# google-research/snap

Measured on AMD Instinct MI355X. Metric: localization_scenes_per_sec, higher is better.
Workload: dtype f32 (tensors, accumulation, every non-GEMM op); conv / dense products on the bf16 matrix cores: operands split into 2 bf16 parts, 3 part products per MAC, ~2^-17 per product; 1 GPU; C2: 8 scenes/GPU, 4 StreetView views @512px + aerial, 128x128x60 voxel BEV @0.2m, ResNet-50 encoders, 10001 pose hypotheses; scenes_per_gpu=8, batches_in_flight=2, global_batch=8, parallelism=scene-sharded x1, no data-path collective, mode=inference forward (BEVLocalizer.apply, train=False)

## Files before the change

### include/snap_hip.h

```cpp
#ifndef SNAP_HIP_H_
#define SNAP_HIP_H_

#include <stddef.h>
#include <stdint.h>

#ifdef __cplusplus
extern "C" {
#endif

typedef enum SnapStatus {
  SNAP_OK = 0,
  SNAP_ERR_BAD_SHAPE = -1,
  SNAP_ERR_UNSUPPORTED = -2,
  SNAP_ERR_NULL = -3,
  SNAP_ERR_LAUNCH = -4,
  SNAP_ERR_WORKSPACE = -5
} SnapStatus;

int snap_abi_version(void);
const char* snap_status_string(int status);
const char* snap_build_arch(void);

enum { SNAP_PRO_NONE = 0, SNAP_PRO_AFFINE = 1, SNAP_PRO_GN_RELU = 2,
       SNAP_PRO_RELU_GN = 3, SNAP_PRO_RELU = 4 };
enum { SNAP_EPI_BIAS = 1, SNAP_EPI_RELU = 2, SNAP_EPI_RESIDUAL = 4,
       SNAP_EPI_UPSAMPLE2X_ADD = 8, SNAP_EPI_ROWMASK = 16,
       SNAP_EPI_GELU = 32  };

typedef struct SnapConvDesc {
  int32_t N, H, W, Cin, Cin_stride;
  int32_t KH, KW, stride, pad_t, pad_l;
  int32_t Ho, Wo, Cout, Cout_stride;
  int32_t prologue;
  int32_t epilogue;
  float in_scale, in_shift;
  int32_t tile_hint;
} SnapConvDesc;

int snap_conv2d_nhwc_f32(const SnapConvDesc* desc, const float* x, const float* w,
                         float* y, const float* gn_mu, const float* gn_sc,
                         const float* gn_beta, const float* bias,
                         const float* residual, const float* up_prev,
                         const uint8_t* row_mask, void* stream);

typedef struct SnapConvExtras {
  const int32_t* rows_in;
  const int32_t* rows_out;
  const int32_t* row_count;
  float* gn_partial;
  size_t gn_partial_bytes;
  int32_t gn_partial_relu;
  void* workspace;
  size_t workspace_bytes;
  const void* w_bf16;
  size_t w_bf16_bytes;
  int32_t w_split_parts;
  int32_t w_split_root;
  float* gn_partial2;
  size_t gn_partial2_bytes;
  int32_t gn_partial2_done;
  int32_t x_presplit;
  int32_t ps_tile;
  int32_t ps_res_init;
  int32_t bk_hint;
  int32_t tune_flags;
  int32_t gn_partial_rows;
  int32_t w_half;
  int32_t x_half;
  void* y_half;
  const float* gnb_x;
  const float* gnb_mu;
  const float* gnb_rstd;
  const float* gnb_gamma;
  const float* gnb_beta;
  int32_t gnb_mode;
} SnapConvExtras;
#define SNAP_TUNE_NO_HALO 1
#define SNAP_TUNE_NO_PLAIN 8
#define SNAP_TUNE_RS_NSPLIT_SHIFT 4
int32_t snap_conv2d_presplit_tile_rows(const SnapConvDesc* desc, int32_t ps_tile);
size_t snap_conv2d_presplit_gn_partial_bytes(const SnapConvDesc* desc, int32_t ps_tile);
size_t snap_conv2d_presplit_workspace_bytes(const SnapConvDesc* desc, int32_t ps_tile);
int32_t snap_conv2d_presplit_supported(const SnapConvDesc* desc);
int snap_gn_norm_split_f32(const float* y, const float* partial, int32_t N, int32_t HW, int32_t C,
                           int32_t groups, float eps, int32_t tile_rows, const float* gamma,
                           const float* beta, void* out, float* mu, float* sc, void* stream);
int snap_presplit_f32(const float* x, int64_t rows, int32_t C, void* out, void* stream);

int snap_conv2d_nhwc_ex_f32(const SnapConvDesc* desc, const float* x, const float* w,
                            float* y, const float* gn_mu, const float* gn_sc,
                            const float* gn_beta, const float* bias,
                            const float* residual, const float* up_prev,
                            const uint8_t* row_mask, const SnapConvExtras* extras,
                            void* stream);
size_t snap_conv2d_packed_weights_split_root_bytes(int32_t Cout, int32_t parts);
int snap_conv2d_pack_weights_split_root_bf16(const float* w , int32_t Cout,
                                             int32_t parts, void* out, size_t out_bytes,
                                             void* stream);
size_t snap_conv2d_packed_weights_bytes(int32_t taps, int32_t Cin, int32_t Cout);
int snap_conv2d_pack_weights_bf16(const float* w, int32_t taps, int32_t Cin, int32_t Cout,
                                  void* out, size_t out_bytes, void* stream);
int snap_conv2d_pack_weights_f16(const float* w, int32_t taps, int32_t Cin, int32_t Cout,
                                 void* out, size_t out_bytes, void* stream);
size_t snap_conv2d_packed_weights_split_bytes(int32_t taps, int32_t Cin, int32_t Cout,
                                              int32_t parts);
int snap_conv2d_pack_weights_split_bf16(const float* w, int32_t taps, int32_t Cin, int32_t Cout,
                                        int32_t parts, void* out, size_t out_bytes, void* stream);
typedef struct SnapPackItem {
  const float* w;
  void* out;
  int32_t taps, Cin, Cout, block_begin;
} SnapPackItem;
int32_t snap_conv2d_pack_weights_split_blocks(int32_t taps, int32_t Cin, int32_t Cout);
int32_t snap_conv2d_pack_weights_blocks(int32_t taps, int32_t Cin, int32_t Cout);
int snap_conv2d_pack_weights_multi_bf16(const SnapPackItem* items, int32_t n_items,
                                        int32_t total_blocks, void* stream);
int snap_conv2d_pack_weights_multi_f16(const SnapPackItem* items, int32_t n_items,
                                       int32_t total_blocks, void* stream);
int snap_conv2d_pack_weights_split_multi_bf16(const SnapPackItem* items, int32_t n_items,
                                              int32_t total_blocks, int32_t parts, void* stream);

int snap_interpolate_nd_f32(const float* array, const int32_t* size, int32_t n, int32_t D,
                            const uint8_t* valid_array, const float* points, int64_t K,
                            float* values, uint8_t* valid, void* stream);
int snap_expectation_nd_f32(const float* pdf, int64_t rows, const int32_t* size, int32_t n,
                            float* out, void* stream);
int snap_occupancy_ray_features_f32(const float* hits, const float* origins, const uint8_t* ray_mask,
                                    int64_t num_rays, int32_t num_samples, float margin, const float* points,
                                    int64_t num_points, int32_t B, const float* volume,
                                    const uint8_t* volume_valid, int32_t X, int32_t Y, int32_t Z, int32_t D,
                                    float cell_size, float* out_points, uint8_t* out_labels,
                                    uint8_t* out_ray_valid, float* features, uint8_t* valid, void* stream);
int32_t snap_occupancy_head_supported(int32_t D, int32_t h1, int32_t h2);
int snap_occupancy_head_f32(const float* hits, const float* origins, const uint8_t* ray_mask, int64_t num_rays,
                            int32_t num_samples, float margin, const float* points, int64_t num_points, int32_t B,
                            const float* volume, const uint8_t* volume_valid, int32_t X, int32_t Y, int32_t Z,
                            int32_t D, float cell_size, const float* w0, const float* b0, int32_t h1,
                            const float* w1, const float* b1, int32_t h2, const float* w_out,
                            const float* b_out, float* out_points, uint8_t* out_labels, uint8_t* out_ray_valid,
                            float* logits, uint8_t* valid, void* stream);
int32_t snap_occupancy_features_vjp_chunk(void);
size_t snap_occupancy_features_vjp_workspace_bytes(int64_t num_points, int32_t B, int32_t X, int32_t Y, int32_t Z,
                                                   int32_t D);
int snap_occupancy_ray_features_vjp_f32(const float* hits, const float* origins, const uint8_t* ray_mask,
                                        int64_t num_rays, int32_t num_samples, float margin, const float* points,
                                        int64_t num_points, int32_t B, int32_t X, int32_t Y, int32_t Z, int32_t D,
                                        float cell_size, const float* d_features, float* d_volume, void* workspace,
                                        size_t workspace_bytes, void* stream);

int snap_semantic_embed_f32(const uint8_t* rasters, int64_t M, int32_t N, const int32_t* idx_road,
                            int32_t nr, const int32_t* idx_other, int32_t no,
                            const float* table_road, const float* table_other, int32_t E,
                            float* out, void* stream);
int snap_semantic_onehot_f32(const uint8_t* rasters, int64_t M, int32_t N, const int32_t* idx_road,
                             int32_t nr, const int32_t* idx_other, int32_t no, float* onehot,
                             int32_t KP, void* stream);

int snap_layer_norm_f32(const float* x, const float* gamma, const float* beta, float* y,
// ... 433 lines not shown
```

### snap_amd/_lib.py

```python
import ctypes
import os

_HERE = os.path.dirname(os.path.abspath(__file__))
LIB_PATH = os.environ.get('SNAP_HIP_LIB') or os.path.join(_HERE, 'lib', 'libsnap_hip.so')

c_int = ctypes.c_int32
c_i64 = ctypes.c_int64
c_u64 = ctypes.c_uint64
c_float = ctypes.c_float
c_size = ctypes.c_size_t
ptr = ctypes.c_void_p


class SnapConvDesc(ctypes.Structure):
  _fields_ = [
      ('N', c_int), ('H', c_int), ('W', c_int), ('Cin', c_int),
      ('Cin_stride', c_int),
      ('KH', c_int), ('KW', c_int), ('stride', c_int), ('pad_t', c_int),
      ('pad_l', c_int),
      ('Ho', c_int), ('Wo', c_int), ('Cout', c_int), ('Cout_stride', c_int),
      ('prologue', c_int), ('epilogue', c_int),
      ('in_scale', c_float), ('in_shift', c_float), ('tile_hint', c_int),
  ]


class SnapConvExtras(ctypes.Structure):
  _fields_ = [
      ('rows_in', ptr), ('rows_out', ptr), ('row_count', ptr), ('gn_partial', ptr),
      ('gn_partial_bytes', c_size), ('gn_partial_relu', c_int),
      ('workspace', ptr), ('workspace_bytes', c_size),
      ('w_bf16', ptr), ('w_bf16_bytes', c_size), ('w_split_parts', c_int), ('w_split_root', c_int),
      ('gn_partial2', ptr), ('gn_partial2_bytes', c_size), ('gn_partial2_done', c_int),
      ('x_presplit', c_int), ('ps_tile', c_int), ('ps_res_init', c_int),
      ('bk_hint', c_int), ('tune_flags', c_int), ('gn_partial_rows', c_int), ('w_half', c_int), ('x_half', c_int), ('y_half', ptr),
      ('gnb_x', ptr), ('gnb_mu', ptr), ('gnb_rstd', ptr), ('gnb_gamma', ptr), ('gnb_beta', ptr), ('gnb_mode', c_int),
  ]


class SnapLiftDesc(ctypes.Structure):
  _fields_ = [
      ('B', c_int), ('V', c_int), ('h', c_int), ('w', c_int), ('C', c_int),
      ('feature_dim', c_int), ('num_bins', c_int), ('N', c_int), ('K', c_int),
      ('fisheye', c_int), ('out_stride', c_int),
      ('depth_min', c_float), ('depth_max', c_float),
      ('max_view_distance', c_float),
      ('weighted', c_int), ('use_variance', c_int), ('add_minmax', c_int),
      ('grid_y', c_int), ('grid_z', c_int), ('valid_rows_only', c_int), ('out_split', c_int),
      ('class_rows', c_int), ('tune_flags', c_int),
  ]


SIGNATURES = {
    'snap_abi_version': (c_int, []),
    'snap_status_string': (ctypes.c_char_p, [c_int]),
    'snap_build_arch': (ctypes.c_char_p, []),
    'snap_conv2d_nhwc_f32': (
        c_int,
        [ctypes.POINTER(SnapConvDesc), ptr, ptr, ptr, ptr, ptr, ptr, ptr, ptr,
         ptr, ptr, ptr],
    ),
    'snap_conv2d_nhwc_ex_f32': (
        c_int,
        [ctypes.POINTER(SnapConvDesc), ptr, ptr, ptr, ptr, ptr, ptr, ptr, ptr,
         ptr, ptr, ctypes.POINTER(SnapConvExtras), ptr],
    ),
    'snap_conv2d_gn_partial_bytes': (c_size, [ctypes.POINTER(SnapConvDesc)]),
    'snap_conv2d_workspace_bytes': (c_size, [ctypes.POINTER(SnapConvDesc)]),
    'snap_conv2d_tile_rows': (c_int, [ctypes.POINTER(SnapConvDesc)]),
    'snap_conv2d_pack_weights_blocks': (c_int, [c_int, c_int, c_int]),
    'snap_conv2d_pack_weights_multi_bf16': (c_int, [ptr, c_int, c_int, ptr]),
    'snap_conv2d_pack_weights_multi_f16': (c_int, [ptr, c_int, c_int, ptr]),
    'snap_conv2d_stationary_kind': (c_int, [ctypes.POINTER(SnapConvDesc), c_int]),
    'snap_conv2d_tile_rows_ex': (c_int, [ctypes.POINTER(SnapConvDesc), c_int]),
    'snap_conv2d_gn_partial_bytes_ex': (c_size, [ctypes.POINTER(SnapConvDesc), c_int]),
    'snap_conv2d_splitk_gn_partial_bytes': (c_size, [ctypes.POINTER(SnapConvDesc)]),
    'snap_conv2d_presplit_tile_rows': (c_int, [ctypes.POINTER(SnapConvDesc), c_int]),
    'snap_conv2d_presplit_gn_partial_bytes': (c_size, [ctypes.POINTER(SnapConvDesc), c_int]),
    'snap_conv2d_presplit_workspace_bytes': (c_size, [ctypes.POINTER(SnapConvDesc), c_int]),
    'snap_conv2d_presplit_supported': (c_int, [ctypes.POINTER(SnapConvDesc)]),
    'snap_gn_norm_split_f32': (
        c_int, [ptr, ptr, c_int, c_int, c_int, c_int, c_float, c_int, ptr, ptr, ptr, ptr, ptr, ptr]),
    'snap_presplit_f32': (c_int, [ptr, c_i64, c_int, ptr, ptr]),
    'snap_interpolate_nd_f32': (c_int, [ptr, ptr, c_int, c_int, ptr, ptr, c_i64, ptr, ptr, ptr]),
    'snap_expectation_nd_f32': (c_int, [ptr, c_i64, ptr, c_int, ptr, ptr]),
    'snap_occupancy_ray_features_f32': (
        c_int, [ptr, ptr, ptr, c_i64, c_int, c_float, ptr, c_i64, c_int, ptr, ptr, c_int, c_int, c_int, c_int,
                c_float, ptr, ptr, ptr, ptr, ptr, ptr]),
    'snap_occupancy_head_supported': (c_int, [c_int, c_int, c_int]),
    'snap_occupancy_head_f32': (
        c_int, [ptr, ptr, ptr, c_i64, c_int, c_float, ptr, c_i64, c_int, ptr, ptr, c_int, c_int, c_int, c_int,
                c_float, ptr, ptr, c_int, ptr, ptr, c_int, ptr, ptr, ptr, ptr, ptr, ptr, ptr, ptr]),
    'snap_occupancy_features_vjp_chunk': (c_int, []),
    'snap_occupancy_features_vjp_workspace_bytes': (c_size, [c_i64, c_int, c_int, c_int, c_int, c_int]),
    'snap_occupancy_ray_features_vjp_f32': (
        c_int, [ptr, ptr, ptr, c_i64, c_int, c_float, ptr, c_i64, c_int, c_int, c_int, c_int, c_int, c_float,
                ptr, ptr, ptr, c_size, ptr]),
    'snap_semantic_embed_f32': (
        c_int, [ptr, c_i64, c_int, ptr, c_int, ptr, c_int, ptr, ptr, c_int, ptr, ptr]),
    'snap_semantic_onehot_f32': (c_int, [ptr, c_i64, c_int, ptr, c_int, ptr, c_int, ptr, c_int, ptr]),
    'snap_voting_fft_workspace_bytes': (c_size, [c_int] * 6),
    'snap_voting_fft_f32': (
        c_int, [ptr, ptr, ptr, ptr, ptr, c_int, c_int, c_int, c_int, c_int, c_int, c_float, c_int, ptr, c_size,
                ptr, ptr]),
    'snap_voting_fft_rotated_f32': (
        c_int, [ptr, ptr, ptr, c_float, ptr, ptr, c_int, c_int, c_int, c_int, c_int, c_float, ptr, c_size, ptr, ptr]),
    'snap_stack_templates_f32': (c_int, [ptr, ptr, c_int, c_int, c_int, c_int, c_int, ptr]),
    'snap_stack_templates_rhwd_f32': (c_int, [ptr, ptr, c_int, c_int, c_int, c_int, c_int, ptr]),
    'snap_pack_stacked_templates_split_bf16': (c_int, [ptr, c_int, c_int, c_int, c_int, c_int, ptr, c_size, ptr]),
    'snap_layer_norm_f32': (c_int, [ptr, ptr, ptr, ptr, c_i64, c_int, c_float, ptr]),
    'snap_attention_bf16_f32': (c_int, [ptr, ptr, c_int, c_int, c_int, c_int, c_float, ptr]),
    'snap_layer_norm_bf16out_f32': (c_int, [ptr, ptr, ptr, ptr, c_i64, c_int, c_float, ptr]),
    'snap_attention_bf16out_f32': (c_int, [ptr, ptr, c_int, c_int, c_int, c_int, c_float, ptr]),
    'snap_attention_bf16io': (c_int, [ptr, ptr, c_int, c_int, c_int, c_int, c_float, ptr]),
    'snap_attention_lse_bf16_f32': (c_int, [ptr, ptr, ptr, c_int, c_int, c_int, c_int, c_float, ptr]),
    'snap_attention_bwd_bf16_f32': (
        c_int, [ptr, ptr, ptr, ptr, ptr, ptr, c_int, c_int, c_int, c_int, c_float, ptr]),
    'snap_layer_norm_bwd_workspace_bytes': (c_size, [c_i64, c_int]),
    'snap_layer_norm_bwd_f32': (
# ... 258 lines not shown
```

### snap_amd/csrc/conv_common.h

```cpp
#ifndef SNAP_CSRC_CONV_COMMON_H_
#define SNAP_CSRC_CONV_COMMON_H_

#include <stdio.h>
#include <stdlib.h>

#include "common.h"

namespace snapconv {
struct ConvArgs {
  SnapConvDesc d;
  const float* x;
  const float* w;
  float* y;
  const float* gn_mu;
  const float* gn_sc;
  const float* gn_beta;
  const float* bias;
  const float* residual;
  const float* up_prev;
  const uint8_t* row_mask;
  const int32_t* rows_in;
  const int32_t* rows_out;
  const int32_t* row_count;
  float* kpartial;
  size_t kpartial_bytes;
  int ksplit;
  int slabs_per_split;
  int tiles_per_split;
  float* gn_partial;
  float* gn_partial2;
  int32_t* gn_partial2_done;
  int gn_relu;
  int gn_rows32;
  int gn_slabs;
  int M;
  int K;
  int ctiles;
  int nk;
  int ncol;
  int bk;
  int no_halo;
  int no_plain;
  int rs_nsplit;
  const void* w_bf16;
  int cin8;
  int half;
  const void* x_half;
  void* y_half;
  const void* x_ps;
  int ps_tile;
  int ps_res_init;
  int ps_parts;
  const float* gnb_x;
  const float* gnb_mu;
  const float* gnb_rstd;
  const float* gnb_gamma;
  const float* gnb_beta;
  int gnb_mode;
};

int launch_bf16(ConvArgs a, hipStream_t s);
int launch_split(ConvArgs a, int parts, hipStream_t s);
int launch_split_root(ConvArgs a, int parts, hipStream_t s);
int launch_ps(ConvArgs a, hipStream_t s);
int stationary_kind(const SnapConvDesc& d, int parts, bool row_lists);
int launch_rs(ConvArgs a, hipStream_t s);
int launch_bs(ConvArgs a, hipStream_t s);
int launch_root_ws(const ConvArgs& a, hipStream_t s);
struct PsTile { int bm, bn, nt; };
PsTile ps_choose_tile(int64_t M, int64_t N, int force);
int ps_ksplit(int64_t M, int Cout, int64_t nk, int bm, int bn, size_t kpartial_bytes);

}

namespace {
using snapconv::ConvArgs;

template <int PRO>
__device__ __forceinline__ float apply_pro(float v, float mu, float sc, float beta, float s,
                                           float t) {
  if constexpr (PRO == SNAP_PRO_AFFINE) return v * s + t;
  if constexpr (PRO == SNAP_PRO_GN_RELU) return snap_relu((v - mu) * sc + beta);
  if constexpr (PRO == SNAP_PRO_RELU_GN) return (snap_relu(v) - mu) * sc + beta;
  if constexpr (PRO == SNAP_PRO_RELU) return snap_relu(v);
  return v;
}

typedef __attribute__((address_space(3))) void lds_void_t;
typedef const __attribute__((address_space(1))) void cglobal_void_t;

__device__ __attribute__((aligned(64))) const float kZeroChunk[16] = {0.f};

__device__ __forceinline__ float snap_gelu_tanh(float x) {
  const float u = 0.7978845608028654f * (x + 0.044715f * x * x * x);
  return x / (1.0f + __expf(-2.0f * u));
}

template <int BM, int BN, bool DUAL = false, int NT = 256, bool SKIP_RES = false, int OUTH = 0, bool GNB = false>
__device__ __forceinline__ void conv_epilogue(const ConvArgs& a,
                                              f32x16 (&acc)[BM / (NT / 4)][BN / 64],
                                              float* smem, int m0, int n0, int Meff, int row_t,
                                              int split) {
  constexpr int WR = NT / 128;
  constexpr int TM = BM / (32 * WR), TN = BN / 64;
  const SnapConvDesc& d = a.d;
  const int tid = threadIdx.x;
  const int lane = tid & 63;
  const int wid = tid >> 6;
  const int wr = wid >> 1, wc = wid & 1;
  const int l31 = lane & 31, lhi = lane >> 5;
  const int HoWo = d.Ho * d.Wo;
  const int epi = d.epilogue;
  const int Hp = d.Ho >> 1, Wp = d.Wo >> 1;
  constexpr int Q = BN / 4;
  constexpr int PER_THREAD = (32 * WR * Q) / NT;
  const bool want_stats = a.gn_partial != nullptr && a.ksplit == 1;
  const int n_first = m0 / HoWo;
  const int m_split = (n_first + 1) * HoWo;
  float gs1[2][4] = {{0.f, 0.f, 0.f, 0.f}, {0.f, 0.f, 0.f, 0.f}};
  float gs2[2][4] = {{0.f, 0.f, 0.f, 0.f}, {0.f, 0.f, 0.f, 0.f}};
  const bool want_relu_too = DUAL && want_stats;
  float hs1[2][4] = {{0.f, 0.f, 0.f, 0.f}, {0.f, 0.f, 0.f, 0.f}};
  float hs2[2][4] = {{0.f, 0.f, 0.f, 0.f}, {0.f, 0.f, 0.f, 0.f}};
  f32x4 vb_mu[2], vb_rs[2], vb_g = {0.f, 0.f, 0.f, 0.f}, vb_b = {0.f, 0.f, 0.f, 0.f};
  const bool gnb = GNB && want_stats && a.gnb_mode != 0;
  if constexpr (GNB) {
    vb_mu[0] = vb_mu[1] = vb_rs[0] = vb_rs[1] = vb_g;
    const int colq = n0 + 4 * (tid % Q);
    if (gnb && colq < d.Cout) {
      vb_g = *reinterpret_cast<const f32x4*>(a.gnb_gamma + colq);
      vb_b = *reinterpret_cast<const f32x4*>(a.gnb_beta + colq);
#pragma unroll
      for (int sl = 0; sl < 2; ++sl) {
        const int64_t so = (int64_t)min(n_first + sl, d.N - 1) * d.Cout + colq;
        vb_mu[sl] = *reinterpret_cast<const f32x4*>(a.gnb_mu + so);
        vb_rs[sl] = *reinterpret_cast<const f32x4*>(a.gnb_rstd + so);
      }
    }
  }
#pragma unroll
  for (int h = 0; h < TM; ++h) {
    if (h > 0) __syncthreads();
#pragma unroll
    for (int j = 0; j < TN; ++j)
#pragma unroll
      for (int r = 0; r < 16; ++r) {
        const int ri = (r & 3) + 8 * (r >> 2) + 4 * lhi;
        smem[(wr * 32 + ri) * BN + wc * (BN / 2) + j * 32 + l31] = acc[h][j][r];
      }
    __syncthreads();
#pragma unroll
    for (int it = 0; it < PER_THREAD; ++it) {
      const int idx = tid + NT * it;
      const int row = idx / Q, q = idx - row * Q;
      const int m = m0 + (row >> 5) * (BM / WR) + h * 32 + (row & 31);
      const int col = n0 + 4 * q;
      if (m >= Meff || col >= d.Cout) continue;
      f32x4 v = *reinterpret_cast<const f32x4*>(smem + row * BN + 4 * q);
      if (a.ksplit > 1) {
        *reinterpret_cast<f32x4*>(a.kpartial + ((int64_t)split * a.M + m) * d.Cout + col) = v;
        continue;
      }
      const int64_t o = (int64_t)(a.rows_out ? a.rows_out[m] : m) * d.Cout_stride + col;
      if (epi & SNAP_EPI_BIAS) {
        const f32x4 bb = *reinterpret_cast<const f32x4*>(a.bias + col);
#pragma unroll
        for (int e = 0; e < 4; ++e) v[e] += bb[e];
      }
      if (!SKIP_RES && (epi & SNAP_EPI_RESIDUAL)) {
        const f32x4 rr = *reinterpret_cast<const f32x4*>(a.residual + o);
#pragma unroll
        for (int e = 0; e < 4; ++e) v[e] += rr[e];
      }
      if (epi & SNAP_EPI_UPSAMPLE2X_ADD) {
        const int n = m / HoWo;
        const int rr = m - n * HoWo;
        const int ho = rr / d.Wo;
        const int wo = rr - ho * d.Wo;
        const float sh = (ho + 0.5f) * 0.5f - 0.5f;
        const float sw = (wo + 0.5f) * 0.5f - 0.5f;
        const float fh = floorf(sh), fw = floorf(sw);
        const float wh_hi = sh - fh, wh_lo = 1.f - wh_hi;
        const float ww_hi = sw - fw, ww_lo = 1.f - ww_hi;
        const int h0 = min(max((int)fh, 0), Hp - 1), h1 = min(max((int)fh + 1, 0), Hp - 1);
        const int w0 = min(max((int)fw, 0), Wp - 1), w1 = min(max((int)fw + 1, 0), Wp - 1);
        const int64_t base = (int64_t)n * Hp * Wp;
        const f32x4 p00 = *reinterpret_cast<const f32x4*>(
            a.up_prev + (base + (int64_t)h0 * Wp + w0) * d.Cout_stride + col);
        const f32x4 p01 = *reinterpret_cast<const f32x4*>(
            a.up_prev + (base + (int64_t)h0 * Wp + w1) * d.Cout_stride + col);
        const f32x4 p10 = *reinterpret_cast<const f32x4*>(
            a.up_prev + (base + (int64_t)h1 * Wp + w0) * d.Cout_stride + col);
        const f32x4 p11 = *reinterpret_cast<const f32x4*>(
            a.up_prev + (base + (int64_t)h1 * Wp + w1) * d.Cout_stride + col);
#pragma unroll
        for (int e = 0; e < 4; ++e) {
          const float c0 = p00[e] * wh_lo + p10[e] * wh_hi;
          const float c1 = p01[e] * wh_lo + p11[e] * wh_hi;
          v[e] += c0 * ww_lo + c1 * ww_hi;
        }
      }
      if (epi & SNAP_EPI_RELU) {
#pragma unroll
        for (int e = 0; e < 4; ++e) v[e] = snap_relu(v[e]);
      }
      if (epi & SNAP_EPI_GELU) {
#pragma unroll
        for (int e = 0; e < 4; ++e) v[e] = snap_gelu_tanh(v[e]);
      }
      if ((epi & SNAP_EPI_ROWMASK) && a.row_mask[m] == 0) v = f32x4{0.f, 0.f, 0.f, 0.f};
      if constexpr (OUTH == 0) {
        *reinterpret_cast<f32x4*>(a.y + o) = v;
      } else {
        if (a.y) *reinterpret_cast<f32x4*>(a.y + o) = v;
        if constexpr (OUTH == 1) {
          typedef __bf16 bf16x4_t __attribute__((ext_vector_type(4)));
          *reinterpret_cast<bf16x4_t*>(static_cast<__bf16*>(a.y_half) + o) = __builtin_convertvector(v, bf16x4_t);
        } else {
          typedef _Float16 f16x4_t __attribute__((ext_vector_type(4)));
          *reinterpret_cast<f16x4_t*>(static_cast<_Float16*>(a.y_half) + o) = __builtin_convertvector(v, f16x4_t);
        }
      }
      if (GNB && gnb) {
        const int sl = m >= m_split ? 1 : 0;
        const f32x4 xv = *reinterpret_cast<const f32x4*>(a.gnb_x + (int64_t)m * d.Cout + col);
#pragma unroll
        for (int e = 0; e < 4; ++e) {
          float xh, dyp;
          if (a.gnb_mode == SNAP_PRO_GN_RELU) {
            xh = (xv[e] - vb_mu[sl][e]) * vb_rs[sl][e];
            dyp = (xh * vb_g[e] + vb_b[e] > 0.f) ? v[e] : 0.f;
          } else {
            xh = (fmaxf(xv[e], 0.f) - vb_mu[sl][e]) * vb_rs[sl][e];
            dyp = v[e];
          }
          gs1[sl][e] += dyp;
          gs2[sl][e] += dyp * xh;
        }
      } else if (want_stats) {
        const int sl = m >= m_split ? 1 : 0;
#pragma unroll
        for (int e = 0; e < 4; ++e) {
          const float t = a.gn_relu ? snap_relu(v[e]) : v[e];
          gs1[sl][e] += t;
          gs2[sl][e] += t * t;
          if constexpr (DUAL) {
            const float r = snap_relu(v[e]);
            hs1[sl][e] += r;
            hs2[sl][e] += r * r;
          }
        }
      }
    }
  }
  if (want_stats) {
    constexpr int RG = NT / Q;
    const int q = tid % Q, rg = tid / Q;
    for (int pass = 0; pass < (want_relu_too ? 2 : 1); ++pass) {
    float* const dst_partial = pass ? a.gn_partial2 : a.gn_partial;
    __syncthreads();
#pragma unroll
    for (int sl = 0; sl < 2; ++sl)
#pragma unroll
      for (int e = 0; e < 4; ++e) {
        smem[((rg * 2 + sl) * BN + 4 * q + e) * 2 + 0] = pass ? hs1[sl][e] : gs1[sl][e];
        smem[((rg * 2 + sl) * BN + 4 * q + e) * 2 + 1] = pass ? hs2[sl][e] : gs2[sl][e];
      }
    __syncthreads();
    for (int i = tid; i < 2 * BN; i += NT) {
      const int sl = i / BN, c = i - sl * BN;
      const int col = n0 + c;
      const int n = n_first + sl;
      const bool live = col < d.Cout && n < d.N && (sl == 0 || (m0 + BM > m_split && m_split < Meff));
      if (!live) continue;
      float t1 = 0.f, t2 = 0.f;
#pragma unroll
      for (int r = 0; r < RG; ++r) {
        t1 += smem[((r * 2 + sl) * BN + c) * 2 + 0];
        t2 += smem[((r * 2 + sl) * BN + c) * 2 + 1];
      }
      const int slab = row_t - (int)(((int64_t)n * HoWo) / BM);
      float* o = dst_partial + (((int64_t)n * a.gn_slabs + slab) * d.Cout + col) * 2;
      o[0] = t1;
      o[1] = t2;
    }
    }
  }
}

__global__ __launch_bounds__(256) void splitk_reduce_kernel(
    const float* __restrict__ partial, int S, int64_t M, int Cout, int Cout_stride, int epi,
    const float* __restrict__ bias, const float* __restrict__ residual,
    const uint8_t* __restrict__ row_mask, float* __restrict__ y) {
  const int Q = Cout >> 2;
  const int64_t i = (int64_t)blockIdx.x * blockDim.x + threadIdx.x;
  if (i >= M * Q) return;
  const int64_t m = i / Q;
  const int col = 4 * (int)(i - m * Q);
  f32x4 v = *reinterpret_cast<const f32x4*>(partial + m * Cout + col);
  int s = 1;
  for (; s + 3 < S; s += 4) {
    f32x4 t[4];
#pragma unroll
    for (int u = 0; u < 4; ++u)
      t[u] = *reinterpret_cast<const f32x4*>(partial + ((int64_t)(s + u) * M + m) * Cout + col);
#pragma unroll
    for (int u = 0; u < 4; ++u)
#pragma unroll
      for (int e = 0; e < 4; ++e) v[e] += t[u][e];
  }
  for (; s < S; ++s) {
    const f32x4 t = *reinterpret_cast<const f32x4*>(partial + ((int64_t)s * M + m) * Cout + col);
#pragma unroll
    for (int e = 0; e < 4; ++e) v[e] += t[e];
  }
  const int64_t o = m * Cout_stride + col;
  if (epi & SNAP_EPI_BIAS) {
    const f32x4 bb = *reinterpret_cast<const f32x4*>(bias + col);
#pragma unroll
    for (int e = 0; e < 4; ++e) v[e] += bb[e];
  }
  if (epi & SNAP_EPI_RESIDUAL) {
    const f32x4 rr = *reinterpret_cast<const f32x4*>(residual + o);
#pragma unroll
    for (int e = 0; e < 4; ++e) v[e] += rr[e];
  }
  if (epi & SNAP_EPI_RELU) {
#pragma unroll
    for (int e = 0; e < 4; ++e) v[e] = snap_relu(v[e]);
  }
  if (epi & SNAP_EPI_GELU) {
#pragma unroll
    for (int e = 0; e < 4; ++e) v[e] = snap_gelu_tanh(v[e]);
  }
  if ((epi & SNAP_EPI_ROWMASK) && row_mask[m] == 0) v = f32x4{0.f, 0.f, 0.f, 0.f};
  *reinterpret_cast<f32x4*>(y + o) = v;
}

__global__ __launch_bounds__(256) void splitk_reduce_stats_kernel(
    const float* __restrict__ partial, int S, int64_t M, int Cout, int epi,
    const float* __restrict__ bias, const float* __restrict__ residual,
    const uint8_t* __restrict__ row_mask, float* __restrict__ y, int HoWo, int N, int gn_slabs,
    int gn_relu, float* __restrict__ gn_partial) {
  __shared__ float red[256 * 16];
  const int Q = Cout >> 2;
  const int QW = Q < 256 ? Q : 256;
  const int PW = 256 / QW;
  const int tq = threadIdx.x % QW, tp = threadIdx.x / QW;
  const int64_t m0 = (int64_t)blockIdx.x * 32;
  const int n_first = (int)(m0 / HoWo);
  const int64_t m_split = (int64_t)(n_first + 1) * HoWo;
  for (int q0 = 0; q0 < Q; q0 += QW) {
    const int q = q0 + tq;
    const int col = 4 * q;
    float s1[2][4] = {{0.f, 0.f, 0.f, 0.f}, {0.f, 0.f, 0.f, 0.f}};
    float s2[2][4] = {{0.f, 0.f, 0.f, 0.f}, {0.f, 0.f, 0.f, 0.f}};
    if (q < Q && tp < PW) {
      constexpr int RB = 8;
      for (int r0 = tp; r0 < 32; r0 += RB * PW) {
        f32x4 v[RB];
        bool ok[RB];
#pragma unroll
        for (int k = 0; k < RB; ++k) {
          const int64_t m = m0 + r0 + k * PW;
          ok[k] = r0 + k * PW < 32 && m < M;
          v[k] = *reinterpret_cast<const f32x4*>(partial + (ok[k] ? m : m0) * Cout + col);
        }
        for (int sp = 1; sp < S; ++sp) {
          f32x4 t[RB];
#pragma unroll
          for (int k = 0; k < RB; ++k)
            t[k] = *reinterpret_cast<const f32x4*>(partial + ((int64_t)sp * M + (ok[k] ? m0 + r0 + k * PW : m0)) * Cout + col);
#pragma unroll
          for (int k = 0; k < RB; ++k)
#pragma unroll
            for (int e = 0; e < 4; ++e) v[k][e] += t[k][e];
        }
        f32x4 bb = {0.f, 0.f, 0.f, 0.f};
        if (epi & SNAP_EPI_BIAS) bb = *reinterpret_cast<const f32x4*>(bias + col);
        f32x4 rr[RB];
        if (epi & SNAP_EPI_RESIDUAL) {
#pragma unroll
          for (int k = 0; k < RB; ++k)
            rr[k] = *reinterpret_cast<const f32x4*>(residual + (ok[k] ? m0 + r0 + k * PW : m0) * Cout + col);
        }
#pragma unroll
        for (int k = 0; k < RB; ++k) {
          if (!ok[k]) continue;
          const int64_t m = m0 + r0 + k * PW;
          const int64_t o = m * Cout + col;
          if (epi & SNAP_EPI_BIAS) {
#pragma unroll
            for (int e = 0; e < 4; ++e) v[k][e] += bb[e];
          }
          if (epi & SNAP_EPI_RESIDUAL) {
#pragma unroll
            for (int e = 0; e < 4; ++e) v[k][e] += rr[k][e];
          }
          if (epi & SNAP_EPI_RELU) {
#pragma unroll
            for (int e = 0; e < 4; ++e) v[k][e] = snap_relu(v[k][e]);
          }
          if (epi & SNAP_EPI_GELU) {
#pragma unroll
            for (int e = 0; e < 4; ++e) v[k][e] = snap_gelu_tanh(v[k][e]);
          }
          if ((epi & SNAP_EPI_ROWMASK) && row_mask[m] == 0) v[k] = f32x4{0.f, 0.f, 0.f, 0.f};
          *reinterpret_cast<f32x4*>(y + o) = v[k];
          const int sl = m >= m_split ? 1 : 0;
#pragma unroll
          for (int e = 0; e < 4; ++e) {
            const float t = gn_relu ? snap_relu(v[k][e]) : v[k][e];
            s1[sl][e] += t;
            s2[sl][e] += t * t;
          }
        }
      }
    }
    __syncthreads();
#pragma unroll
    for (int sl = 0; sl < 2; ++sl)
#pragma unroll
      for (int e = 0; e < 4; ++e) {
        red[threadIdx.x * 16 + sl * 8 + e] = s1[sl][e];
        red[threadIdx.x * 16 + sl * 8 + 4 + e] = s2[sl][e];
      }
    __syncthreads();
    if (tp == 0 && q < Q) {
#pragma unroll
      for (int sl = 0; sl < 2; ++sl) {
        const int n = n_first + sl;
        const bool live = n < N && (sl == 0 || (m0 + 32 > m_split && m_split < M));
        if (!live) continue;
        const int slab = (int)(blockIdx.x - (((int64_t)n * HoWo) >> 5));
        float* o = gn_partial + (((int64_t)n * gn_slabs + slab) * Cout + col) * 2;
#pragma unroll
        for (int e = 0; e < 4; ++e) {
          float t1 = 0.f, t2 = 0.f;
          for (int pp = 0; pp < PW; ++pp) {
            t1 += red[(pp * QW + tq) * 16 + sl * 8 + e];
            t2 += red[(pp * QW + tq) * 16 + sl * 8 + 4 + e];
          }
          o[2 * e] = t1;
          o[2 * e + 1] = t2;
        }
      }
    }
  }
}

inline int launch_splitk_reduce(const ConvArgs& a, hipStream_t s) {
  if (a.gn_partial) {
    if (!a.gn_rows32 || (a.d.Cout & 3) || (256 % ((a.d.Cout >> 2) < 256 ? (a.d.Cout >> 2) : 256)) != 0)
      return SNAP_ERR_UNSUPPORTED;
    hipLaunchKernelGGL(splitk_reduce_stats_kernel, dim3((unsigned)snap_cdiv((int64_t)a.M, 32)), dim3(256), 0, s,
                       (const float*)a.kpartial, a.ksplit, (int64_t)a.M, a.d.Cout, a.d.epilogue, a.bias,
                       a.residual, a.row_mask, a.y, a.d.Ho * a.d.Wo, a.d.N, (a.d.Ho * a.d.Wo) / 32 + 2,
                       a.gn_relu, a.gn_partial);
  } else {
    const int64_t total4 = (int64_t)a.M * (a.d.Cout / 4);
    hipLaunchKernelGGL(splitk_reduce_kernel, dim3((unsigned)snap_cdiv(total4, 256)), dim3(256), 0, s,
                       (const float*)a.kpartial, a.ksplit, (int64_t)a.M, a.d.Cout, a.d.Cout_stride,
                       a.d.epilogue, a.bias, a.residual, a.row_mask, a.y);
  }
  SNAP_CHECK_LAUNCH();
  return SNAP_OK;
}

constexpr int64_t splitk_max_tiles() { return 384; }
constexpr int splitk_target() { return 768; }

struct TileChoice { int bm, bn; };
inline int hint_tile(int h) { return h % 1000000; }
inline int hint_mode(int h) { return h / 1000000; }
inline int64_t desc_k(const SnapConvDesc& d) { return (int64_t)d.KH * d.KW * d.Cin; }
inline TileChoice choose_tile(int64_t M, int64_t N, int forced, int64_t K) {
  forced = hint_tile(forced);
  const int64_t kMin = 512;
  const bool n_wide_ok = N > 64 && !(N % 128 != 0 && N % 128 <= 64);
  if (forced != 128128 && forced != 128064 && forced != 64128 && forced != 64064) forced = 0;
  if (forced == 128128 || (!forced && n_wide_ok && snap_cdiv(M, 128) * snap_cdiv(N, 128) >= kMin))
    return {128, 128};
  if (!forced && n_wide_ok && K >= 2304 && M >= 128) return {128, 128};
  const int64_t t64128 = snap_cdiv(M, 64) * snap_cdiv(N, 128);
  if (!forced && n_wide_ok && N >= 512 && K >= 1024 && t64128 >= kMin) return {64, 128};
  if (forced == 128064 || (!forced && snap_cdiv(M, 128) * snap_cdiv(N, 64) >= kMin)) return {128, 64};
  if (forced == 64128 || (!forced && n_wide_ok && N >= 512 && t64128 >= kMin)) return {64, 128};
  if (!forced && n_wide_ok && K >= 1024 && t64128 >= 256) return {64, 128};
  return {64, 64};
}

}

#endif
```

### snap_amd/csrc/conv_igemm.hip

```cpp
#include "conv_common.h"

namespace {

template <int BM, int BN, bool VEC, int PRO, int BK, bool DMA = false>
__device__ __forceinline__ void conv_igemm_body(const ConvArgs& a) {
  constexpr int AS = BM + 2;
  constexpr int TM = BM / 64;
  constexpr int TN = BN / 64;
  constexpr int QPR = BK / 4;
  constexpr int RPP = 256 / QPR;
  constexpr int AROWS = BM / RPP;
  constexpr int SRPP = 256 / BK;
  constexpr int AELEMS = BM / SRPP;
  constexpr int BQ = BN / 4;
  constexpr int BROWS_PER_PASS = 256 / BQ;
  constexpr int BPASS = BK / BROWS_PER_PASS;

  constexpr int kDmaStages = 3;
  constexpr int kSlabFloats = DMA ? kDmaStages * (BK * BM + BK * BN) : 2 * BK * AS + 2 * BK * BN;
  constexpr int kStageFloats = 64 * BN;
  constexpr int kSmemFloats = kSlabFloats > kStageFloats ? kSlabFloats : kStageFloats;
  __shared__ __attribute__((aligned(16))) float smem[kSmemFloats];
  float* const As0 = smem;
  float* const Bs0 = smem + 2 * BK * AS;
// ... 246 lines not shown
          const int R = wr * (BM / 2) + i * 32 + l31;
          const int pq = (lhi * 2 + h) ^ ((R >> 2) & 3);
          av[i][h] = *reinterpret_cast<const f32x4*>(as + 4 * (R * 4 + pq));
          if constexpr (PRO == SNAP_PRO_RELU) {
#pragma unroll
            for (int e = 0; e < 4; ++e) av[i][h][e] = snap_relu(av[i][h][e]);
          }
        }
      float bv[2][TN];
#pragma unroll
      for (int jn = 0; jn < TN; ++jn) bv[0][jn] = bs[(8 * lhi) * BN + wc * (BN / 2) + jn * 32 + l31];
#pragma unroll
      for (int j = 0; j < BK / 2; ++j) {
        const int cu = j & 1, nx = cu ^ 1;
        if (j + 1 < BK / 2) {
#pragma unroll
          for (int jn = 0; jn < TN; ++jn)
            bv[nx][jn] = bs[(8 * lhi + j + 1) * BN + wc * (BN / 2) + jn * 32 + l31];
        }
#pragma unroll
        for (int i = 0; i < TM; ++i)
#pragma unroll
          for (int jn = 0; jn < TN; ++jn)
            acc[i][jn] = __builtin_amdgcn_mfma_f32_32x32x2f32(av[i][j >> 2][j & 3], bv[cu][jn], acc[i][jn], 0, 0, 0);
      }
      __builtin_amdgcn_sched_group_barrier(0x100, 2 * TM + TN, 0);
#pragma unroll
      for (int j = 0; j < BK / 2; ++j) {
        if (j + 1 < BK / 2) __builtin_amdgcn_sched_group_barrier(0x100, TN, 0);
        __builtin_amdgcn_sched_group_barrier(0x008, TM * TN, 0);
      }
    }
    __syncthreads();
  } else {
  load_slab(kt_begin);
  advance();
  store_slab(0);
  __syncthreads();

  for (int kt = kt_begin; kt < kt_end; ++kt) {
    const int cur = (kt - kt_begin) & 1;
    const bool more = kt + 1 < kt_end;
    if (more) {
      load_slab(kt + 1);
      advance();
    }
    const float* as = As0 + cur * (BK * AS);
    const float* bs = Bs0 + cur * (BK * BN);
    float av[2][TM], bv[2][TN];
#pragma unroll
    for (int i = 0; i < TM; ++i) av[0][i] = as[lhi * AS + wr * (BM / 2) + i * 32 + l31];
#pragma unroll
    for (int j = 0; j < TN; ++j) bv[0][j] = bs[lhi * BN + wc * (BN / 2) + j * 32 + l31];
#pragma unroll
    for (int kk = 0; kk < BK / 2; ++kk) {
      const int cu = kk & 1, nx = cu ^ 1;
      if (kk + 1 < BK / 2) {
#pragma unroll
        for (int i = 0; i < TM; ++i)
          av[nx][i] = as[(2 * (kk + 1) + lhi) * AS + wr * (BM / 2) + i * 32 + l31];
#pragma unroll
        for (int j = 0; j < TN; ++j)
          bv[nx][j] = bs[(2 * (kk + 1) + lhi) * BN + wc * (BN / 2) + j * 32 + l31];
      }
#pragma unroll
      for (int i = 0; i < TM; ++i)
#pragma unroll
        for (int j = 0; j < TN; ++j)
          acc[i][j] =
              __builtin_amdgcn_mfma_f32_32x32x2f32(av[cu][i], bv[cu][j], acc[i][j], 0, 0, 0);
    }
    __builtin_amdgcn_sched_group_barrier(0x100, TM + TN, 0);
#pragma unroll
    for (int kk = 0; kk < BK / 2; ++kk) {
      if (kk + 1 < BK / 2) __builtin_amdgcn_sched_group_barrier(0x100, TM + TN, 0);
      __builtin_amdgcn_sched_group_barrier(0x008, TM * TN, 0);
    }
    if (more) store_slab(cur ^ 1);
    __syncthreads();
  }

  }

  conv_epilogue<BM, BN>(a, acc, smem, m0, n0, Meff, row_t, split);
}


template <int BM, int BN, bool VEC, int PRO, int BK>
__global__ __launch_bounds__(256) void conv_igemm_kernel(const ConvArgs a) {
  conv_igemm_body<BM, BN, VEC, PRO, BK>(a);
}
template <int BM, int BN, bool VEC, int PRO, int BK>
__global__ __launch_bounds__(256) __attribute__((amdgpu_waves_per_eu(4, 4)))
void conv_igemm_kernel_occ4(const ConvArgs a) {
  conv_igemm_body<BM, BN, VEC, PRO, BK>(a);
}
template <int BM, int BN, int PRO>
__global__ __launch_bounds__(256) void conv_igemm_kernel_dma(const ConvArgs a) {
  conv_igemm_body<BM, BN, true, PRO, 16, true>(a);
}

template <int BM, int BN, bool VEC, int PRO, int BK>
int launch(ConvArgs a, hipStream_t s) {
  if (VEC) {
    a.ctiles = (a.d.Cin + BK - 1) / BK;
    a.nk = a.d.KH * a.d.KW * a.ctiles;
  } else {
    a.ctiles = 0;
    a.nk = (a.K + BK - 1) / BK;
  }
  const int64_t nrow = snap_cdiv(a.M, BM);
  a.ncol = (int)snap_cdiv(a.d.Cout, BN);
  a.gn_slabs = (a.d.Ho * a.d.Wo) / BM + 2;
  int64_t nblocks = snap_cdiv(nrow, 8) * 8 * a.ncol;
  if (nblocks > 0x7fffffffLL) return SNAP_ERR_BAD_SHAPE;
  a.ksplit = 1;
  a.tiles_per_split = (int)nblocks;
  a.slabs_per_split = a.nk;
  const int64_t tiles = nrow * a.ncol;
  const int target = splitk_target();
  if (a.kpartial && target > 0 && tiles <= splitk_max_tiles() && a.nk >= 16 && !a.rows_in &&
      !a.rows_out && !a.row_count && !a.gn_partial &&
      !(a.d.epilogue & SNAP_EPI_UPSAMPLE2X_ADD)) {
    int64_t S = (target + tiles - 1) / tiles;
    S = S < a.nk / 8 ? S : a.nk / 8;
    const int64_t fit = (int64_t)(a.kpartial_bytes / ((size_t)a.M * a.d.Cout * sizeof(float)));
    S = S < fit ? S : fit;
    if (S >= 2) {
      a.slabs_per_split = (int)((a.nk + S - 1) / S);
      a.ksplit = (a.nk + a.slabs_per_split - 1) / a.slabs_per_split;
      nblocks *= a.ksplit;
    }
  }
  constexpr bool kGn = PRO == SNAP_PRO_GN_RELU || PRO == SNAP_PRO_RELU_GN;
  constexpr bool kDmaOk = VEC && BK == 16 && (PRO == SNAP_PRO_NONE || PRO == SNAP_PRO_RELU);
  bool launched = false;
  if constexpr (kDmaOk) {
    hipLaunchKernelGGL((conv_igemm_kernel_dma<BM, BN, PRO>), dim3((unsigned)nblocks), dim3(256), 0,
                       s, a);
    launched = true;
  }
  if (launched) {
  } else if constexpr (!kGn && BK == 16 && (VEC || BM * BN < 128 * 128)) {
    hipLaunchKernelGGL((conv_igemm_kernel_occ4<BM, BN, VEC, PRO, BK>), dim3((unsigned)nblocks),
                       dim3(256), 0, s, a);
  } else {
    hipLaunchKernelGGL((conv_igemm_kernel<BM, BN, VEC, PRO, BK>), dim3((unsigned)nblocks),
                       dim3(256), 0, s, a);
  }
  SNAP_CHECK_LAUNCH();
  if (a.ksplit > 1) {
    const int64_t total4 = (int64_t)a.M * (a.d.Cout / 4);
    hipLaunchKernelGGL(splitk_reduce_kernel, dim3((unsigned)snap_cdiv(total4, 256)), dim3(256), 0, s,
                       (const float*)a.kpartial, a.ksplit, (int64_t)a.M, a.d.Cout, a.d.Cout_stride,
                       a.d.epilogue, a.bias, a.residual, a.row_mask, a.y);
    SNAP_CHECK_LAUNCH();
  }
  return SNAP_OK;
}

template <int BM, int BN, bool VEC, int BK>
int launch_pro(const ConvArgs& a, hipStream_t s) {
  switch (a.d.prologue) {
    case SNAP_PRO_NONE: return launch<BM, BN, VEC, SNAP_PRO_NONE, BK>(a, s);
    case SNAP_PRO_AFFINE: return launch<BM, BN, VEC, SNAP_PRO_AFFINE, BK>(a, s);
    case SNAP_PRO_GN_RELU:
      if constexpr (VEC) return launch<BM, BN, VEC, SNAP_PRO_GN_RELU, BK>(a, s);
// ... 109 lines not shown
  return (size_t)d.N * (HoWo / t.bm + 2) * d.Cout * 2 * sizeof(float);
}

extern "C" size_t snap_conv2d_presplit_workspace_bytes(const SnapConvDesc* desc, int32_t ps_tile) {
  if (!desc) return 0;
  const SnapConvDesc& d = *desc;
  if (d.Cin % 16 != 0 || (d.epilogue & SNAP_EPI_UPSAMPLE2X_ADD)) return 0;
  const int64_t M = (int64_t)d.N * d.Ho * d.Wo;
  const snapconv::PsTile t = snapconv::ps_choose_tile(M, d.Cout, ps_tile);
  const int64_t nk = (int64_t)d.KH * d.KW * (d.Cin / 16);
  const int S = snapconv::ps_ksplit(M, d.Cout, nk, t.bm, t.bn, (size_t)-1);
  return S >= 2 ? (size_t)S * M * d.Cout * sizeof(float) : 0;
}

extern "C" int snap_conv2d_nhwc_ex_f32(const SnapConvDesc* desc, const float* x,
                                       const float* w, float* y, const float* gn_mu,
                                       const float* gn_sc, const float* gn_beta,
                                       const float* bias, const float* residual,
                                       const float* up_prev, const uint8_t* row_mask,
                                       const SnapConvExtras* ex, void* stream) {
  if (!desc || !x || !w || (!y && !(ex && ex->y_half))) return SNAP_ERR_NULL;
  const int32_t* rows_in = ex ? ex->rows_in : nullptr;
  const int32_t* rows_out = ex ? ex->rows_out : nullptr;
  const int32_t* row_count = ex ? ex->row_count : nullptr;
  float* gn_partial = ex ? ex->gn_partial : nullptr;
  if ((rows_in || rows_out) &&
      (desc->epilogue & (SNAP_EPI_RESIDUAL | SNAP_EPI_UPSAMPLE2X_ADD | SNAP_EPI_ROWMASK)))
    return SNAP_ERR_UNSUPPORTED;
  if (ex && (ex->tune_flags & 2)) return SNAP_ERR_UNSUPPORTED;
  const bool presplit = ex && ex->x_presplit;
  const bool split_vec = ex && ex->w_bf16 && !ex->w_split_root && !rows_in && !rows_out && !row_count;
  const bool rows32 = gn_partial && ex->gn_partial_rows == 32;
  if (gn_partial && ex->gn_partial_rows != 0 && ex->gn_partial_rows != 32) return SNAP_ERR_BAD_SHAPE;
  if (rows32 && (presplit || !split_vec || ex->w_split_parts == 1 || !ex->workspace || ex->gn_partial2 ||
                 ex->y_half || ex->gnb_mode))
    return SNAP_ERR_UNSUPPORTED;
  const size_t gn_need = !gn_partial ? 0
                         : rows32    ? snap_conv2d_splitk_gn_partial_bytes(desc)
                         : presplit  ? snap_conv2d_presplit_gn_partial_bytes(desc, ex->ps_tile)
                                     : snap_conv2d_gn_partial_bytes_ex(desc, split_vec ? ex->w_split_parts : 0);
  if (gn_partial) {
    if (rows_in || rows_out || row_count) return SNAP_ERR_UNSUPPORTED;
    if (desc->Cout_stride != desc->Cout) return SNAP_ERR_UNSUPPORTED;
    if (ex->gn_partial_bytes < gn_need || gn_need == 0) return SNAP_ERR_WORKSPACE;
  }
  const SnapConvDesc& d = *desc;
  if (d.N <= 0 || d.H <= 0 || d.W <= 0 || d.Cin <= 0 || d.Cout <= 0 || d.KH <= 0 ||
      d.KW <= 0 || d.stride <= 0 || d.Ho <= 0 || d.Wo <= 0)
    return SNAP_ERR_BAD_SHAPE;
  if (d.Cin_stride < d.Cin || d.Cout_stride < d.Cout) return SNAP_ERR_BAD_SHAPE;
  if (d.Cout % 4 != 0 || d.Cout_stride % 4 != 0) return SNAP_ERR_BAD_SHAPE;
  if ((reinterpret_cast<uintptr_t>(y) & 15) || (reinterpret_cast<uintptr_t>(w) & 15) ||
      (reinterpret_cast<uintptr_t>(bias) & 15) || (reinterpret_cast<uintptr_t>(residual) & 15) ||
      (reinterpret_cast<uintptr_t>(up_prev) & 15))
    return SNAP_ERR_BAD_SHAPE;
  if ((int64_t)d.N * d.Ho * d.Wo > 0x7fffffffLL) return SNAP_ERR_BAD_SHAPE;
  const bool gn = d.prologue == SNAP_PRO_GN_RELU || d.prologue == SNAP_PRO_RELU_GN;
  if (d.prologue < 0 || d.prologue > SNAP_PRO_RELU) return SNAP_ERR_UNSUPPORTED;
  if (gn && (!gn_mu || !gn_sc || !gn_beta)) return SNAP_ERR_NULL;
  if ((d.epilogue & SNAP_EPI_BIAS) && !bias) return SNAP_ERR_NULL;
  if ((d.epilogue & SNAP_EPI_RESIDUAL) && !residual) return SNAP_ERR_NULL;
  if ((d.epilogue & SNAP_EPI_ROWMASK) && !row_mask) return SNAP_ERR_NULL;
  if (d.epilogue & SNAP_EPI_UPSAMPLE2X_ADD) {
    if (!up_prev) return SNAP_ERR_NULL;
    if ((d.Ho & 1) || (d.Wo & 1)) return SNAP_ERR_BAD_SHAPE;
  }
  ConvArgs a;
  a.d = d;
  a.x = x; a.w = w; a.y = y;
  a.gn_mu = gn_mu; a.gn_sc = gn_sc; a.gn_beta = gn_beta;
  a.bias = bias; a.residual = residual; a.up_prev = up_prev; a.row_mask = row_mask;
  a.rows_in = rows_in; a.rows_out = rows_out; a.row_count = row_count;
  a.gn_partial = gn_partial;
  a.gn_relu = ex ? ex->gn_partial_relu : 0;
  a.gn_rows32 = rows32 ? 1 : 0;
  a.gn_partial2 = nullptr;
  a.gn_partial2_done = nullptr;
  if (gn_partial && ex->gn_partial2) {
    if (a.gn_relu || ex->gn_partial2_bytes < gn_need) return SNAP_ERR_WORKSPACE;
    a.gn_partial2 = ex->gn_partial2;
    a.gn_partial2_done = const_cast<int32_t*>(&ex->gn_partial2_done);
    *a.gn_partial2_done = 0;
  }
  a.kpartial = ex ? static_cast<float*>(ex->workspace) : nullptr;
  a.kpartial_bytes = ex ? ex->workspace_bytes : 0;
  if (reinterpret_cast<uintptr_t>(a.kpartial) & 15) a.kpartial = nullptr;
  a.ksplit = 1; a.slabs_per_split = 0; a.tiles_per_split = 0;
  a.gn_slabs = 0;
  a.M = d.N * d.Ho * d.Wo;
  a.K = d.KH * d.KW * d.Cin;
  const bool vec = (d.Cin_stride % 4 == 0) && (d.Cin >= 4) &&
                   ((reinterpret_cast<uintptr_t>(x) & 15) == 0) &&
                   (!gn || (d.Cin % 4 == 0));
  a.ctiles = 0;
  a.nk = 0;
  a.bk = (ex && ex->bk_hint == 32) ? 32 : 16;
  a.no_halo = (ex && (ex->tune_flags & SNAP_TUNE_NO_HALO)) ? 1 : 0;
  a.rs_nsplit = ex ? (ex->tune_flags >> SNAP_TUNE_RS_NSPLIT_SHIFT) & 15 : 0;
  a.no_plain = (ex && (ex->tune_flags & SNAP_TUNE_NO_PLAIN)) ? 1 : 0;
  hipStream_t s = static_cast<hipStream_t>(stream);
  a.w_bf16 = ex ? ex->w_bf16 : nullptr;
  a.half = (ex && ex->w_half) ? 1 : 0;
  if (a.half && (ex->w_split_parts != 0 || presplit || ex->w_split_root)) return SNAP_ERR_UNSUPPORTED;
  a.x_half = nullptr;
  a.y_half = nullptr;
  const bool ps1 = presplit && ex->w_split_parts == 1;
  if (ex && ex->y_half) {
    if (!a.w_bf16 || (ex->w_split_parts != 0 && !ps1) || (presplit && !ps1) || ex->w_split_root || gn_partial ||
        (d.epilogue & SNAP_EPI_UPSAMPLE2X_ADD) || d.Cout_stride % 4 != 0 ||
        (reinterpret_cast<uintptr_t>(ex->y_half) & 7))
      return SNAP_ERR_UNSUPPORTED;
    a.y_half = ex->y_half;
    a.kpartial = nullptr;
  }
  a.gnb_x = a.gnb_mu = a.gnb_rstd = a.gnb_gamma = a.gnb_beta = nullptr;
  a.gnb_mode = 0;
  if (ex && ex->gnb_mode) {
    if ((ex->gnb_mode != SNAP_PRO_GN_RELU && ex->gnb_mode != SNAP_PRO_RELU_GN) || !ex->x_half || !gn_partial ||
        ex->gn_partial_rows != 0 || ex->gn_partial2 || ex->gn_partial_relu || ex->workspace ||
        (d.epilogue & ~(SNAP_EPI_RESIDUAL | SNAP_EPI_BIAS)))
      return SNAP_ERR_UNSUPPORTED;
    if (!ex->gnb_x || !ex->gnb_mu || !ex->gnb_rstd || !ex->gnb_gamma || !ex->gnb_beta) return SNAP_ERR_NULL;
    if ((reinterpret_cast<uintptr_t>(ex->gnb_x) | reinterpret_cast<uintptr_t>(ex->gnb_mu) |
         reinterpret_cast<uintptr_t>(ex->gnb_rstd) | reinterpret_cast<uintptr_t>(ex->gnb_gamma) |
         reinterpret_cast<uintptr_t>(ex->gnb_beta)) & 15)
      return SNAP_ERR_BAD_SHAPE;
    a.gnb_x = ex->gnb_x; a.gnb_mu = ex->gnb_mu; a.gnb_rstd = ex->gnb_rstd;
    a.gnb_gamma = ex->gnb_gamma; a.gnb_beta = ex->gnb_beta;
    a.gnb_mode = ex->gnb_mode;
  }
  a.cin8 = (d.Cin + 7) / 8 * 8;
  a.x_ps = nullptr;
  a.ps_tile = 0;
  a.ps_res_init = 0;
  a.ps_parts = 2;
  if (ex && ex->x_half) {
    if (!a.w_bf16 || ex->w_split_parts != 0 || presplit || ex->w_split_root || d.prologue != SNAP_PRO_NONE ||
        rows_in || d.Cin_stride % 8 != 0 || d.Cin % 8 != 0 || ex->y_half)
      return SNAP_ERR_UNSUPPORTED;
    if (ex->w_bf16_bytes < snap_conv2d_packed_weights_bytes(d.KH * d.KW, d.Cin, d.Cout)) return SNAP_ERR_WORKSPACE;
    if ((reinterpret_cast<uintptr_t>(a.w_bf16) | reinterpret_cast<uintptr_t>(x)) & 15) return SNAP_ERR_BAD_SHAPE;
    a.x_half = x;
    a.x = nullptr;
    return snapconv::launch_bf16(a, s);
  }
  if (presplit) {
    if (!a.w_bf16 || (ex->w_split_parts != 2 && ex->w_split_parts != 1) || ex->w_split_root) return SNAP_ERR_UNSUPPORTED;
    if (ps1 && d.Cin_stride != d.Cin) return SNAP_ERR_UNSUPPORTED;
    a.ps_parts = ex->w_split_parts;
    const size_t need = snap_conv2d_packed_weights_split_bytes(d.KH * d.KW, d.Cin, d.Cout, ex->w_split_parts);
    if (need == 0) return SNAP_ERR_UNSUPPORTED;
    if (ex->w_bf16_bytes < need) return SNAP_ERR_WORKSPACE;
    if ((reinterpret_cast<uintptr_t>(a.w_bf16) | reinterpret_cast<uintptr_t>(x)) & 15) return SNAP_ERR_BAD_SHAPE;
    a.x_ps = x;
    a.x = nullptr;
    a.ps_tile = ex->ps_tile;
    a.ps_res_init = ex->ps_res_init;
    a.cin8 = d.Cin;
    return snapconv::launch_ps(a, s);
  }
  if (a.w_bf16 && ex->w_split_root) {
    const int parts = ex->w_split_parts;
    if (ex->w_bf16_bytes < snap_conv2d_packed_weights_split_root_bytes(d.Cout, parts) ||
        snap_conv2d_packed_weights_split_root_bytes(d.Cout, parts) == 0)
      return SNAP_ERR_WORKSPACE;
    if ((reinterpret_cast<uintptr_t>(a.w_bf16) | reinterpret_cast<uintptr_t>(x)) & 15) return SNAP_ERR_BAD_SHAPE;
    a.cin8 = 16;
    return snapconv::launch_split_root(a, parts, s);
  }
  if (a.w_bf16 && vec) {
    const int parts = ex->w_split_parts;
    if (parts < 0 || parts == 1 || parts > 3) return SNAP_ERR_UNSUPPORTED;
    const size_t need = parts ? snap_conv2d_packed_weights_split_bytes(d.KH * d.KW, d.Cin, d.Cout, parts)
                              : snap_conv2d_packed_weights_bytes(d.KH * d.KW, d.Cin, d.Cout);
    if (need == 0) return SNAP_ERR_UNSUPPORTED;
    if (ex->w_bf16_bytes < need) return SNAP_ERR_WORKSPACE;
    if (parts) a.cin8 = (d.Cin + 15) / 16 * 16;
    if (reinterpret_cast<uintptr_t>(a.w_bf16) & 15) return SNAP_ERR_BAD_SHAPE;
    return parts ? snapconv::launch_split(a, parts, s) : snapconv::launch_bf16(a, s);
  }
  return vec ? launch_tile<true>(a, s) : launch_tile<false>(a, s);
}
```

### snap_amd/csrc/conv_split.hip

```cpp
#include "conv_common.h"

namespace {

typedef __bf16 bf16x8 __attribute__((ext_vector_type(8)));
typedef __bf16 bf16x4 __attribute__((ext_vector_type(4)));

typedef unsigned u32x2 __attribute__((ext_vector_type(2)));
typedef unsigned u32x4 __attribute__((ext_vector_type(4)));

template <int NS>
__device__ __forceinline__ void split_bf16(const f32x4& v, u32x2 (&out)[NS]) {
  typedef __bf16 bf16x2 __attribute__((ext_vector_type(2)));
  typedef float f32x2 __attribute__((ext_vector_type(2)));
  f32x4 r = v;
#pragma unroll
  for (int p = 0; p < NS; ++p) {
#pragma unroll
    for (int h = 0; h < 2; ++h) {
      const f32x2 pr = {r[2 * h], r[2 * h + 1]};
      const bf16x2 b = __builtin_convertvector(pr, bf16x2);
      unsigned u;
      __builtin_memcpy(&u, &b, 4);
      out[p][h] = u;
      if (p + 1 < NS) {
// ... 214 lines not shown
        else
          v[e] = xin[i] ? pv : 0.f;
      }
      u32x2 parts[NS];
      split_bf16<NS>(v, parts);
      const int oct = (akq >> 1) ^ ((row >> 3) & 1);
      char* dst = Ab + buf * A_ST + row * 32 + oct * 16 + (akq & 1) * 8;
#pragma unroll
      for (int p = 0; p < NS; ++p) *reinterpret_cast<u32x2*>(dst + p * A_PART) = parts[p];
    }
  };

  const int l31 = lane & 31, lhi = lane >> 5;
  int g_ct = ct;
  auto next_gct = [&]() { if (++g_ct == a.ctiles) g_ct = 0; };
  int ring_cur = 0;
  if (kt_begin < kt_end) {
    if constexpr (gn_tab) {
      issue_gn(0, g_ct); next_gct();
      issue_gn(1, g_ct); next_gct();
    }
    load_a();
    issue_b(0);
    advance();
    if constexpr (gn_tab) {
      asm volatile("s_waitcnt vmcnt(0)" ::: "memory");
      __syncthreads();
    }
    store_a(0, 0);
    asm volatile("s_waitcnt vmcnt(0)" ::: "memory");
    __syncthreads();
  }
  for (int kt = kt_begin; kt < kt_end; ++kt) {
    const int cur = (kt - kt_begin) & 1;
    const bool more = kt + 1 < kt_end;
    const int ring_next = ring_cur == 2 ? 0 : ring_cur + 1;
    if (more) {
      load_a();
      issue_b(cur ^ 1);
      advance();
      if constexpr (gn_tab) {
        if (kt + 2 < kt_end) { issue_gn(ring_next == 2 ? 0 : ring_next + 1, g_ct); next_gct(); }
      }
    }
    const char* as = Ab + cur * A_ST;
    const char* bs = Bb + cur * B_ST;
    bf16x8 av[TM][NS], bv[TN][NS];
#pragma unroll
    for (int i = 0; i < TM; ++i) {
      const int R = wr * (BM / 2) + i * 32 + l31;
      const char* p0 = as + R * 32 + ((lhi ^ ((R >> 3) & 1)) * 16);
#pragma unroll
      for (int p = 0; p < NS; ++p) av[i][p] = *reinterpret_cast<const bf16x8*>(p0 + p * A_PART);
    }
#pragma unroll
    for (int j = 0; j < TN; ++j) {
      const int C = wc * (BN / 2) + j * 32 + l31;
      const char* p0 = bs + C * 32 + ((lhi ^ ((C >> 3) & 1)) * 16);
#pragma unroll
      for (int p = 0; p < NS; ++p) bv[j][p] = *reinterpret_cast<const bf16x8*>(p0 + p * B_PART);
    }
#define SNAP_SPLIT_PRODUCT(PA, PB)                                                          \
  _Pragma("unroll") for (int i = 0; i < TM; ++i) _Pragma("unroll") for (int j = 0; j < TN; ++j) \
      acc[i][j] = __builtin_amdgcn_mfma_f32_32x32x16_bf16(av[i][PA], bv[j][PB], acc[i][j], 0, 0, 0);
    if constexpr (NS == 3) {
      SNAP_SPLIT_PRODUCT(2, 0)
      SNAP_SPLIT_PRODUCT(0, 2)
      SNAP_SPLIT_PRODUCT(1, 1)
      SNAP_SPLIT_PRODUCT(1, 0)
      SNAP_SPLIT_PRODUCT(0, 1)
      SNAP_SPLIT_PRODUCT(0, 0)
    } else {
      SNAP_SPLIT_PRODUCT(1, 0)
      SNAP_SPLIT_PRODUCT(0, 1)
      SNAP_SPLIT_PRODUCT(0, 0)
    }
#undef SNAP_SPLIT_PRODUCT
    if (more) store_a(cur ^ 1, ring_next);
    ring_cur = ring_next;
    asm volatile("s_waitcnt vmcnt(0)" ::: "memory");
    __syncthreads();
  }

  conv_epilogue<BM, BN, DUAL>(a, acc, smem, m0, n0, Meff, row_t, split);
}

template <int BN, int PRO, int NS, int HPMAX>
__device__ __forceinline__ void conv3x3_halo_body(const ConvArgs& a) {
  constexpr int BM = 128, BK = 16;
  constexpr int TM = 2, TN = BN / 64;
  constexpr int NPER = (HPMAX * 4 + 255) / 256;
  constexpr int H_PART = HPMAX * 32;
  constexpr int H_ST = NS * H_PART;
  constexpr int B_PART = BN * 32;
  constexpr int B_ST = NS * B_PART;
  constexpr int BSLOTS = NS * BN * 2;
  constexpr int BPIECES = (BSLOTS + 255) / 256;
  constexpr int kSlabBytes = 2 * (H_ST + B_ST);
  constexpr int kStageBytes = 64 * BN * 4;
  constexpr int kSmemBytes = kSlabBytes > kStageBytes ? kSlabBytes : kStageBytes;
  constexpr bool need_gn = (PRO == SNAP_PRO_GN_RELU || PRO == SNAP_PRO_RELU_GN);
  constexpr int kGnRing = 320;
  __shared__ __attribute__((aligned(16))) float smem[(kSmemBytes + (need_gn ? 2 * kGnRing : 0)) / 4];
  char* const Hb = reinterpret_cast<char*>(smem);
  char* const Bb = Hb + 2 * H_ST;
  char* const Gt = Hb + kSmemBytes;

  const SnapConvDesc& d = a.d;
  const int tid = threadIdx.x;
  const int lane = tid & 63;
  const int wid = tid >> 6;
  const int wr = wid >> 1, wc = wid & 1;
  const int l31 = lane & 31, lhi = lane >> 5;
  const int ncol = a.ncol;
  const int split = a.ksplit > 1 ? blockIdx.x / a.tiles_per_split : 0;
  const int bid = a.ksplit > 1 ? blockIdx.x - split * a.tiles_per_split : blockIdx.x;
  const int xcd = bid & 7;
  const int seq = bid >> 3;
  const int col_t = seq % ncol;
  const int row_t = (seq / ncol) * 8 + xcd;
  const int Meff = a.M;
  if (row_t * BM >= Meff) return;
  const int m0 = row_t * BM;
  const int n0 = col_t * BN;
  const int W = d.W, HW = d.H * d.W;
  const int n_first = m0 / HW;
  const int m_split = (n_first + 1) * HW;
  const int n_second = min(n_first + 1, d.N - 1);
  const int halo0 = m0 - W - 1;
  const int HP = BM + 2 * W + 2;

  int tapmask[TM];
#pragma unroll
  for (int i = 0; i < TM; ++i) {
    const int m = m0 + wr * 64 + i * 32 + l31;
    int mk = 0;
    if (m < Meff) {
      const int r = m % HW;
      const int y = r / W, x = r - y * W;
#pragma unroll
      for (int t = 0; t < 9; ++t) {
        const int yy = y + t / 3 - 1, xx = x + t % 3 - 1;
        if (yy >= 0 && yy < d.H && xx >= 0 && xx < W) mk |= 1 << t;
      }
    }
    tapmask[i] = mk;
  }

  const int Mtot = d.N * HW;
  auto halo_ok_row = [&](int hp) {
    const int mp = halo0 + hp;
    return hp < HP && mp >= 0 && mp < Mtot;
  };
  f32x4 xa[NPER];
  auto load_halo = [&](int ct) {
#pragma unroll
    for (int j = 0; j < NPER; ++j) {
      const int f = tid + 256 * j;
      const int hp = f >> 2;
      const bool ok = halo_ok_row(hp);
      const float* px = a.x + ((int64_t)(ok ? halo0 + hp : 0) * d.Cin_stride + 4 * (f & 3) + ct * BK);
      xa[j] = *reinterpret_cast<const f32x4*>(ok ? px : a.x);
    }
  };
  auto issue_gn = [&](int ring, int ct) {
    if constexpr (need_gn) {
      if (tid < 20) {
// ... 66 lines not shown
  for (int i = 0; i < TM; ++i)
#pragma unroll
    for (int j = 0; j < TN; ++j)
#pragma unroll
      for (int r = 0; r < 16; ++r) acc[i][j][r] = 0.f;

  const int ct_begin = a.ksplit > 1 ? split * a.slabs_per_split : 0;
  const int ct_end = a.ksplit > 1 ? min(ctiles, ct_begin + a.slabs_per_split) : ctiles;
  issue_gn(0, ct_begin);
  load_halo(ct_begin);
  issue_b(0, ct_begin, 0);
  if constexpr (need_gn) {
    asm volatile("s_waitcnt vmcnt(0)" ::: "memory");
    __syncthreads();
  }
  store_halo(0, 0);
  asm volatile("s_waitcnt vmcnt(0)" ::: "memory");
  __syncthreads();

  int bcur = 0;
  for (int ct = ct_begin; ct < ct_end; ++ct) {
    const int hb = (ct - ct_begin) & 1;
    const bool more_ct = ct + 1 < ct_end;
#pragma unroll 1
    for (int t = 0; t < 9; ++t) {
      const bool last = !more_ct && t == 8;
      const bool fetch = t == 0 && more_ct;
      if (fetch) issue_gn(hb ^ 1, ct + 1);
      if (!last) issue_b(bcur ^ 1, t == 8 ? ct + 1 : ct, t == 8 ? 0 : t + 1);
      if (fetch) {
        asm volatile("" ::: "memory");
        load_halo(ct + 1);
        asm volatile("" ::: "memory");
      }
      const int kh = t / 3, kw = t - 3 * kh;
      const int toff = kh * W + kw;
      const char* hs = Hb + hb * H_ST;
      const char* bs = Bb + bcur * B_ST;
      bf16x8 av[TM][NS], bv[TN][NS];
#pragma unroll
      for (int i = 0; i < TM; ++i) {
        const int h = wr * 64 + i * 32 + l31 + toff;
        const char* p0 = hs + h * 32 + ((lhi ^ ((h >> 3) & 1)) * 16);
        const bool in = (tapmask[i] >> t) & 1;
#pragma unroll
        for (int p = 0; p < NS; ++p) {
          u32x4 raw = *reinterpret_cast<const u32x4*>(p0 + p * H_PART);
          if (!in) raw = u32x4{0u, 0u, 0u, 0u};
          __builtin_memcpy(&av[i][p], &raw, 16);
        }
      }
#pragma unroll
      for (int j = 0; j < TN; ++j) {
        const int C = wc * (BN / 2) + j * 32 + l31;
        const char* p0 = bs + C * 32 + ((lhi ^ ((C >> 3) & 1)) * 16);
#pragma unroll
        for (int p = 0; p < NS; ++p) bv[j][p] = *reinterpret_cast<const bf16x8*>(p0 + p * B_PART);
      }
#define SNAP_SPLIT_PRODUCT(PA, PB)                                                          \
  _Pragma("unroll") for (int i = 0; i < TM; ++i) _Pragma("unroll") for (int j = 0; j < TN; ++j) \
      acc[i][j] = __builtin_amdgcn_mfma_f32_32x32x16_bf16(av[i][PA], bv[j][PB], acc[i][j], 0, 0, 0);
      if constexpr (NS == 3) {
        SNAP_SPLIT_PRODUCT(2, 0)
        SNAP_SPLIT_PRODUCT(0, 2)
        SNAP_SPLIT_PRODUCT(1, 1)
        SNAP_SPLIT_PRODUCT(1, 0)
        SNAP_SPLIT_PRODUCT(0, 1)
        SNAP_SPLIT_PRODUCT(0, 0)
      } else {
        SNAP_SPLIT_PRODUCT(1, 0)
        SNAP_SPLIT_PRODUCT(0, 1)
        SNAP_SPLIT_PRODUCT(0, 0)
      }
#undef SNAP_SPLIT_PRODUCT
      if (t == 2 && more_ct) store_halo(hb ^ 1, hb ^ 1);
      if (fetch)
        asm volatile("s_waitcnt vmcnt(%0)" ::"n"(NPER) : "memory");
      else
        asm volatile("s_waitcnt vmcnt(0)" ::: "memory");
      asm volatile("s_waitcnt lgkmcnt(0)\n\ts_barrier" ::: "memory");
      bcur ^= 1;
    }
  }
  conv_epilogue<BM, BN>(a, acc, smem, m0, n0, Meff, row_t, split);
}

template <int BN, int PRO, int NS, int HPMAX>
__global__ __launch_bounds__(256, NS == 2 ? 3 : 2) void conv3x3_halo_kernel(const ConvArgs a) {
  conv3x3_halo_body<BN, PRO, NS, HPMAX>(a);
}

inline bool halo_ok(const ConvArgs& a) {
  const bool on = !a.no_halo;
  const SnapConvDesc& d = a.d;
  const int hp = 128 + 2 * d.W + 2;
  return on && d.KH == 3 && d.KW == 3 && d.stride == 1 && d.pad_t == 1 && d.pad_l == 1 &&
         d.Ho == d.H && d.Wo == d.W && d.Cin % 16 == 0 && !a.rows_in && !a.rows_out &&
         !a.row_count && hp <= 288 && d.H * d.W >= hp &&
         (int64_t)d.N * d.H * d.W * d.Cin_stride < 0x7fffffffLL &&
         (d.prologue == SNAP_PRO_GN_RELU || d.prologue == SNAP_PRO_NONE);
}

template <int BN, int PRO, int NS>
void launch_halo(const ConvArgs& a, dim3 grid, hipStream_t s) {
  const int hp = 128 + 2 * a.d.W + 2;
  if (hp <= 208)
    hipLaunchKernelGGL((conv3x3_halo_kernel<BN, PRO, NS, 208>), grid, dim3(256), 0, s, a);
  else
    hipLaunchKernelGGL((conv3x3_halo_kernel<BN, PRO, NS, 288>), grid, dim3(256), 0, s, a);
}

template <int BM, int BN, int PRO, int NS, bool GNT, bool TAIL, bool DUAL = false, bool PLAIN = false>
__global__ __launch_bounds__(256, NS == 2 ? 4 : 3) void conv_split_kernel(const ConvArgs a) {
  conv_split_body<BM, BN, PRO, NS, GNT, TAIL, false, DUAL, PLAIN>(a);
}

template <int BN, int PRO, int NS>
__global__ __launch_bounds__(256, NS == 2 ? 4 : 3) void conv_split_root_kernel(const ConvArgs a) {
  conv_split_body<128, BN, PRO, NS, false, false, true>(a);
}

template <int BM, int BN, int PRO, int NS>
int launch(ConvArgs a, hipStream_t s) {
  constexpr int BK = 16;
  a.ctiles = (a.d.Cin + BK - 1) / BK;
  a.nk = a.d.KH * a.d.KW * a.ctiles;
  const int64_t nrow = snap_cdiv(a.M, BM);
  a.ncol = (int)snap_cdiv(a.d.Cout, BN);
  a.gn_slabs = (a.d.Ho * a.d.Wo) / BM + 2;
  int64_t nblocks = snap_cdiv(nrow, 8) * 8 * a.ncol;
  if (nblocks > 0x7fffffffLL) return SNAP_ERR_BAD_SHAPE;
  a.ksplit = 1;
  a.tiles_per_split = (int)nblocks;
  a.slabs_per_split = a.nk;
  const int64_t tiles = nrow * a.ncol;
  const int target = splitk_target();
  if (a.kpartial && target > 0 && tiles <= splitk_max_tiles() && a.nk >= 16 && !a.rows_in &&
      !a.rows_out && !a.row_count && (!a.gn_partial || (a.gn_rows32 && a.d.Cout_stride == a.d.Cout)) &&
      !(a.d.epilogue & SNAP_EPI_UPSAMPLE2X_ADD)) {
    int64_t S = (target + tiles - 1) / tiles;
    S = S < a.nk / 8 ? S : a.nk / 8;
    const int64_t fit = (int64_t)(a.kpartial_bytes / ((size_t)a.M * a.d.Cout * sizeof(float)));
    S = S < fit ? S : fit;
    if (S >= 2) {
      a.slabs_per_split = (int)((a.nk + S - 1) / S);
      a.ksplit = (a.nk + a.slabs_per_split - 1) / a.slabs_per_split;
      nblocks *= a.ksplit;
    }
  }
  if (a.gn_partial && a.gn_rows32 && a.ksplit == 1) return SNAP_ERR_WORKSPACE;
  constexpr bool need_gn = (PRO == SNAP_PRO_GN_RELU || PRO == SNAP_PRO_RELU_GN);
  const bool table_ok = !need_gn || (a.d.Ho * a.d.Wo >= BM && !a.rows_in);
  const bool tail = (a.d.Cin & 3) != 0;
  const dim3 grid((unsigned)nblocks);
  if constexpr (BM == 128 && (PRO == SNAP_PRO_GN_RELU || PRO == SNAP_PRO_NONE)) {
    if (halo_ok(a)) {
      if (a.ksplit > 1) {
        const int per = (a.ctiles + a.ksplit - 1) / a.ksplit;
        ConvArgs h = a;
        h.slabs_per_split = per;
        h.ksplit = (a.ctiles + per - 1) / per;
        if (h.ksplit > 1) {
          const dim3 hgrid((unsigned)(h.tiles_per_split * h.ksplit));
          launch_halo<BN, PRO, NS>(h, hgrid, s);
          SNAP_CHECK_LAUNCH();
          return launch_splitk_reduce(h, s);
        }
// ... 105 lines not shown
    const SnapPackItem* __restrict__ items, int n_items, int parts) {
  int lo = 0, hi = n_items - 1;
  while (lo < hi) {
    const int mid = (lo + hi + 1) >> 1;
    if (items[mid].block_begin <= (int)blockIdx.x) lo = mid; else hi = mid - 1;
  }
  const SnapPackItem it = items[lo];
  const int ctiles = (it.Cin + 15) / 16;
  const int gx = (16 * ctiles + 31) / 32;
  const int gy = ((it.Cout + 127) / 128 * 128) / 32;
  const int local = blockIdx.x - it.block_begin;
  const int t = local / (gx * gy);
  const int rem = local - t * (gx * gy);
  pack_weights_split_body(it.w, static_cast<__bf16*>(it.out), it.taps, it.Cin, ctiles, it.Cout, parts,
                          rem % gx, rem / gx, t);
}

__global__ __launch_bounds__(256) void pack_weights_split_root_kernel(const float* __restrict__ w,
                                                                      __bf16* __restrict__ out,
                                                                      int Cout, int cout128, int parts) {
  const int i = blockIdx.x * 256 + threadIdx.x;
  if (i >= 14 * cout128 * 16) return;
  const int k = i & 15;
  const int n = (i >> 4) % cout128;
  const int t = i / (16 * cout128);
  const int kh = t >> 1, kw = 4 * (t & 1) + (k >> 2), c = k & 3;
  float r = (kw < 7 && c < 3 && n < Cout) ? w[((kh * 7 + kw) * 3 + c) * Cout + n] : 0.f;
  const int col = n & 127;
  const int oct = (k >> 3) ^ ((col >> 3) & 1);
  __bf16* o = out + ((int64_t)(n >> 7) * 14 + t) * ((int64_t)parts * 2048) + col * 16 + oct * 8 + (k & 7);
  for (int p = 0; p < parts; ++p) {
    const __bf16 b = (__bf16)r;
    o[p * 2048] = b;
    r -= (float)b;
  }
}

}

namespace {
template <int BN, int NS>
int launch_root_pro(const ConvArgs& a, dim3 grid, hipStream_t s) {
  if (a.d.prologue == SNAP_PRO_AFFINE)
    hipLaunchKernelGGL((conv_split_root_kernel<BN, SNAP_PRO_AFFINE, NS>), grid, dim3(256), 0, s, a);
  else if (a.d.prologue == SNAP_PRO_NONE)
    hipLaunchKernelGGL((conv_split_root_kernel<BN, SNAP_PRO_NONE, NS>), grid, dim3(256), 0, s, a);
  else
    return SNAP_ERR_UNSUPPORTED;
  SNAP_CHECK_LAUNCH();
  return SNAP_OK;
}
}

int snapconv::launch_split_root(ConvArgs a, int parts, hipStream_t s) {
  const SnapConvDesc& d = a.d;
  if (d.KH != 7 || d.KW != 7 || d.stride != 2 || d.pad_t != 3 || d.pad_l != 3 || d.Cin != 3 ||
      d.Cin_stride != 4 || a.rows_in || a.rows_out || a.row_count || a.gn_partial)
    return SNAP_ERR_UNSUPPORTED;
  if (parts == 2 && d.Cout == 64 && d.Cout_stride == 64 && hint_mode(d.tile_hint) != 1 &&
      (d.prologue == SNAP_PRO_AFFINE || d.prologue == SNAP_PRO_NONE) && !(d.epilogue & ~SNAP_EPI_RELU) &&
      (a.M >= 40000 || hint_mode(d.tile_hint) == 2 || hint_mode(d.tile_hint) == 4) && d.W >= 8)
    return launch_root_ws(a, s);
  a.d.KW = 2;
  a.ctiles = 1;
  a.nk = 14;
  a.ksplit = 1;
  a.slabs_per_split = a.nk;
  const bool wide = d.Cout > 64;
  const int bn = wide ? 128 : 64;
  a.ncol = (int)snap_cdiv(d.Cout, bn);
  a.gn_slabs = (d.Ho * d.Wo) / 128 + 2;
  const int64_t nblocks = snap_cdiv(snap_cdiv(a.M, 128), 8) * 8 * a.ncol;
  if (nblocks > 0x7fffffffLL) return SNAP_ERR_BAD_SHAPE;
  a.tiles_per_split = (int)nblocks;
  const dim3 grid((unsigned)nblocks);
  if (parts == 2) return wide ? launch_root_pro<128, 2>(a, grid, s) : launch_root_pro<64, 2>(a, grid, s);
  if (parts == 3) return wide ? launch_root_pro<128, 3>(a, grid, s) : launch_root_pro<64, 3>(a, grid, s);
  return SNAP_ERR_UNSUPPORTED;
}

int snapconv::launch_split(ConvArgs a, int parts, hipStream_t s) {
  const int kind = stationary_kind(a.d, parts, a.rows_in || a.rows_out || a.row_count);
  if (kind && a.gn_partial && a.gn_rows32) return SNAP_ERR_WORKSPACE;
  switch (kind) {
    case 1: return launch_rs(a, s);
    case 2: case 3: return launch_bs(a, s);
    default: break;
  }
  if (parts == 2) return launch_tile<2>(a, s);
  if (parts == 3) return launch_tile<3>(a, s);
  return SNAP_ERR_UNSUPPORTED;
}

extern "C" size_t snap_conv2d_packed_weights_split_bytes(int32_t taps, int32_t Cin, int32_t Cout,
                                                         int32_t parts) {
  if (parts < 1 || parts > 3 || taps <= 0 || Cin <= 0 || Cout <= 0) return 0;
  const size_t cin16 = ((size_t)Cin + 15) / 16 * 16;
  const size_t cout128 = ((size_t)Cout + 127) / 128 * 128;
  const size_t elems = (size_t)parts * cout128 * taps * cin16;
  if (elems >= ((size_t)1 << 33)) return 0;
  return elems * 2;
}

extern "C" int snap_conv2d_pack_weights_split_bf16(const float* w, int32_t taps, int32_t Cin,
                                                   int32_t Cout, int32_t parts, void* out,
                                                   size_t out_bytes, void* stream) {
  if (!w || !out) return SNAP_ERR_NULL;
  if (taps <= 0 || Cin <= 0 || Cout <= 0) return SNAP_ERR_BAD_SHAPE;
  if (parts < 1 || parts > 3) return SNAP_ERR_UNSUPPORTED;
  const size_t need = snap_conv2d_packed_weights_split_bytes(taps, Cin, Cout, parts);
  if (need == 0) return SNAP_ERR_UNSUPPORTED;
  if (out_bytes < need) return SNAP_ERR_WORKSPACE;
  if (reinterpret_cast<uintptr_t>(out) & 15) return SNAP_ERR_BAD_SHAPE;
  const int ctiles = (Cin + 15) / 16;
  const int cout128 = (Cout + 127) / 128 * 128;
  const dim3 grid((unsigned)snap_cdiv(16 * ctiles, 32), (unsigned)(cout128 / 32), (unsigned)taps);
  hipLaunchKernelGGL(pack_weights_split_kernel, grid, dim3(256), 0, static_cast<hipStream_t>(stream),
                     w, static_cast<__bf16*>(out), taps, Cin, ctiles, Cout, parts);
  SNAP_CHECK_LAUNCH();
  return SNAP_OK;
}

extern "C" int32_t snap_conv2d_pack_weights_split_blocks(int32_t taps, int32_t Cin, int32_t Cout) {
  if (taps <= 0 || Cin <= 0 || Cout <= 0) return 0;
  const int ctiles = (Cin + 15) / 16;
  return ((16 * ctiles + 31) / 32) * (((Cout + 127) / 128 * 128) / 32) * taps;
}

extern "C" int snap_conv2d_pack_weights_split_multi_bf16(const SnapPackItem* items, int32_t n_items,
                                                         int32_t total_blocks, int32_t parts,
                                                         void* stream) {
  if (!items) return SNAP_ERR_NULL;
  if (n_items <= 0 || total_blocks <= 0) return SNAP_ERR_BAD_SHAPE;
  if (parts < 1 || parts > 3) return SNAP_ERR_UNSUPPORTED;
  hipLaunchKernelGGL(pack_weights_split_multi_kernel, dim3((unsigned)total_blocks), dim3(256), 0,
                     static_cast<hipStream_t>(stream), items, n_items, parts);
  SNAP_CHECK_LAUNCH();
  return SNAP_OK;
}

extern "C" size_t snap_conv2d_packed_weights_split_root_bytes(int32_t Cout, int32_t parts) {
  if (parts < 2 || parts > 3 || Cout <= 0) return 0;
  return (size_t)parts * ((Cout + 127) / 128 * 128) * 14 * 16 * 2;
}

extern "C" int snap_conv2d_pack_weights_split_root_bf16(const float* w, int32_t Cout, int32_t parts,
                                                        void* out, size_t out_bytes, void* stream) {
  if (!w || !out) return SNAP_ERR_NULL;
  const size_t need = snap_conv2d_packed_weights_split_root_bytes(Cout, parts);
  if (need == 0) return SNAP_ERR_UNSUPPORTED;
  if (out_bytes < need) return SNAP_ERR_WORKSPACE;
  if (reinterpret_cast<uintptr_t>(out) & 15) return SNAP_ERR_BAD_SHAPE;
  const int cout128 = (Cout + 127) / 128 * 128;
  hipLaunchKernelGGL(pack_weights_split_root_kernel, dim3((unsigned)snap_cdiv(14 * cout128 * 16, 256)),
                     dim3(256), 0, static_cast<hipStream_t>(stream), w, static_cast<__bf16*>(out),
                     Cout, cout128, parts);
  SNAP_CHECK_LAUNCH();
  return SNAP_OK;
}
```

### snap_amd/csrc/encoder_ops.hip

```cpp
#include "common.h"

namespace {

constexpr int WS_COLS = 32;
constexpr int WS_SLICES = 32;

__device__ __forceinline__ void weight_std_body(const float* __restrict__ w,
                                                float* __restrict__ out, int K, int Cout,
                                                float eps, int blk) {
  __shared__ float red[2][WS_SLICES][WS_COLS + 1];
  __shared__ float stat[2][WS_COLS];
  const int tc = threadIdx.x % WS_COLS, tk = threadIdx.x / WS_COLS;
  const int col = blk * WS_COLS + tc;
  const bool ok = col < Cout;
  const float piv = ok ? w[col] : 0.f;
  float s1 = 0.f, s2 = 0.f;
  if (ok)
    for (int k = tk; k < K; k += WS_SLICES) {
      const float t = w[(int64_t)k * Cout + col] - piv;
      s1 += t;
      s2 += t * t;
    }
  red[0][tk][tc] = s1;
  red[1][tk][tc] = s2;
  __syncthreads();
  if (tk == 0) {
    double t1 = 0.0, t2 = 0.0;
#pragma unroll
    for (int i = 0; i < WS_SLICES; ++i) {
      t1 += (double)red[0][i][tc];
      t2 += (double)red[1][i][tc];
    }
    const double m = t1 / (double)K;
    const double var = t2 / (double)K - m * m;
    stat[0][tc] = (float)((double)piv + m);
    stat[1][tc] = sqrtf((float)fmax(var, 0.0) + eps);
  }
  __syncthreads();
  const float mean = stat[0][tc];
  const float denom = stat[1][tc];
  if (ok)
    for (int k = tk; k < K; k += WS_SLICES) {
      const int64_t o = (int64_t)k * Cout + col;
      out[o] = (w[o] - mean) / denom;
    }
}

constexpr int WS4_SLICES = 128;

__device__ __forceinline__ void weight_std_body_v4(const float* __restrict__ w, float* __restrict__ out,
                                                   int K, int Cout, float eps, int blk) {
  __shared__ float red4[2][WS4_SLICES][WS_COLS + 1];
  __shared__ float stat4[2][WS_COLS];
  const int tq = threadIdx.x & 7, tk = threadIdx.x >> 3;
  const int col0 = blk * WS_COLS + 4 * tq;
  const bool ok = col0 < Cout;
  const f32x4 piv = ok ? *reinterpret_cast<const f32x4*>(w + col0) : f32x4{0.f, 0.f, 0.f, 0.f};
  float s1[4] = {0.f, 0.f, 0.f, 0.f}, s2[4] = {0.f, 0.f, 0.f, 0.f};
  if (ok) {
    int k = tk;
    for (; k + 3 * WS4_SLICES < K; k += 4 * WS4_SLICES) {
      f32x4 v[4];
#pragma unroll
      for (int u = 0; u < 4; ++u)
        v[u] = *reinterpret_cast<const f32x4*>(w + (int64_t)(k + u * WS4_SLICES) * Cout + col0);
#pragma unroll
      for (int u = 0; u < 4; ++u)
#pragma unroll
        for (int e = 0; e < 4; ++e) {
          const float t = v[u][e] - piv[e];
          s1[e] += t;
          s2[e] += t * t;
        }
    }
    for (; k < K; k += WS4_SLICES) {
      const f32x4 v = *reinterpret_cast<const f32x4*>(w + (int64_t)k * Cout + col0);
#pragma unroll
      for (int e = 0; e < 4; ++e) {
        const float t = v[e] - piv[e];
        s1[e] += t;
        s2[e] += t * t;
      }
    }
// ... 23 lines not shown
#pragma unroll
    for (int e = 0; e < 4; ++e) { mean[e] = stat4[0][4 * tq + e]; denom[e] = stat4[1][4 * tq + e]; }
    for (int k = tk; k < K; k += WS4_SLICES) {
      const int64_t o = (int64_t)k * Cout + col0;
      const f32x4 v = *reinterpret_cast<const f32x4*>(w + o);
      f32x4 r;
#pragma unroll
      for (int e = 0; e < 4; ++e) r[e] = (v[e] - mean[e]) / denom[e];
      *reinterpret_cast<f32x4*>(out + o) = r;
    }
  }
}

__device__ __forceinline__ bool weight_std_quads_ok(const float* w, const float* out, int Cout) {
  return (Cout & 3) == 0 && ((reinterpret_cast<uintptr_t>(w) | reinterpret_cast<uintptr_t>(out)) & 15) == 0;
}

__global__ __launch_bounds__(1024) void weight_std_kernel(const float* __restrict__ w,
                                                          float* __restrict__ out, int K,
                                                          int Cout, float eps) {
  if (weight_std_quads_ok(w, out, Cout)) weight_std_body_v4(w, out, K, Cout, eps, blockIdx.x);
  else weight_std_body(w, out, K, Cout, eps, blockIdx.x);
}

__global__ __launch_bounds__(1024) void weight_std_multi_kernel(const SnapWstdItem* __restrict__ items,
                                                                int n_items, float eps) {
  int lo = 0, hi = n_items - 1;
  while (lo < hi) {
    const int mid = (lo + hi + 1) >> 1;
    if (items[mid].block_begin <= (int)blockIdx.x) lo = mid; else hi = mid - 1;
  }
  const SnapWstdItem it = items[lo];
  if (weight_std_quads_ok(it.w, it.out, it.Cout)) weight_std_body_v4(it.w, it.out, it.K, it.Cout, eps, blockIdx.x - it.block_begin);
  else weight_std_body(it.w, it.out, it.K, it.Cout, eps, blockIdx.x - it.block_begin);
}

__global__ __launch_bounds__(256) void gn_partial_kernel(
    const float* __restrict__ x, int HW, int C, int Cs, int relu_first, int ppb,
    float* __restrict__ partial ) {
  __shared__ float part[256 * 8];
  const int S = gridDim.x;
  const int n = blockIdx.y;
  const int cbase = blockIdx.z * 1024;
  const int cchunk = min(C - cbase, 1024);
  const int QW = cchunk >> 2;
  const int PW = 256 / QW;
  const int tq = threadIdx.x % QW, tp = threadIdx.x / QW;
  const int c0 = cbase + 4 * tq;
  const int p_begin = blockIdx.x * ppb;
  const int p_end = min(p_begin + ppb, HW);
  const float* xb = x + ((int64_t)n * HW) * Cs + c0;
  f32x4 piv = *reinterpret_cast<const f32x4*>(xb);
  if (relu_first) {
#pragma unroll
    for (int e = 0; e < 4; ++e) piv[e] = snap_relu(piv[e]);
  }
  float s1[4] = {0.f, 0.f, 0.f, 0.f}, s2[4] = {0.f, 0.f, 0.f, 0.f};
  for (int p = p_begin + tp; p < p_end; p += PW) {
    const f32x4 v = *reinterpret_cast<const f32x4*>(xb + (int64_t)p * Cs);
#pragma unroll
    for (int e = 0; e < 4; ++e) {
      const float t = (relu_first ? snap_relu(v[e]) : v[e]) - piv[e];
      s1[e] += t;
      s2[e] += t * t;
    }
  }
#pragma unroll
  for (int e = 0; e < 4; ++e) {
    part[threadIdx.x * 8 + e] = s1[e];
    part[threadIdx.x * 8 + 4 + e] = s2[e];
  }
  __syncthreads();
  for (int c = threadIdx.x; c < cchunk; c += 256) {
    const int q = c >> 2, e = c & 3;
    float a1 = 0.f, a2 = 0.f;
    for (int pp = 0; pp < PW; ++pp) {
      a1 += part[(pp * QW + q) * 8 + e];
      a2 += part[(pp * QW + q) * 8 + 4 + e];
    }
    float* o = partial + (((int64_t)n * S + blockIdx.x) * C + cbase + c) * 2;
    o[0] = a1;
    o[1] = a2;
  }
}

__device__ __forceinline__ double wave_sum_f64(double v) {
#pragma unroll
  for (int o = 32; o > 0; o >>= 1) v += __shfl_xor(v, o, 64);
  return v;
}

__global__ __launch_bounds__(256) void gn_finalize_kernel(
    const float* __restrict__ x, const float* __restrict__ partial, int S, int HW, int C, int Cs,
    int groups, int relu_first, float eps, const float* __restrict__ gamma,
    float* __restrict__ mu, float* __restrict__ sc, float* __restrict__ rstd_out, int total,
    int tile_rows) {
  const int lane = threadIdx.x & 63;
  const int i = blockIdx.x * 4 + (threadIdx.x >> 6);
  if (i >= total) return;
  const int n = i / groups, g = i - n * groups;
  const int cpg = C / groups;
  const int c_lo = g * cpg;
  const bool tiled = tile_rows > 0;
  const float* xp = tiled ? nullptr : x + ((int64_t)n * HW) * Cs + c_lo;
  double t1 = 0.0, t2 = 0.0, u = 0.0, p1 = 0.0, p2 = 0.0;
  int live = S;
  if (tiled)
    live = (int)((((int64_t)(n + 1) * HW - 1) / tile_rows) - (((int64_t)n * HW) / tile_rows)) + 1;
  const int count = live * cpg;
  for (int e = lane; e < count; e += 64) {
    const int s = e / cpg, cc = e - s * cpg;
    float pv = tiled ? 0.f : xp[cc];
    if (relu_first && !tiled) pv = snap_relu(pv);
    const float* pp = partial + (((int64_t)n * S + s) * C + c_lo + cc) * 2;
    const double a1 = (double)pp[0];
    t1 += a1;
    t2 += (double)pp[1];
    u += (double)pv * a1;
  }
  for (int cc = lane; cc < cpg && !tiled; cc += 64) {
    float pv = xp[cc];
    if (relu_first) pv = snap_relu(pv);
    p1 += (double)pv;
    p2 += (double)pv * (double)pv;
  }
  t1 = wave_sum_f64(t1); t2 = wave_sum_f64(t2); u = wave_sum_f64(u);
  p1 = wave_sum_f64(p1); p2 = wave_sum_f64(p2);
  const double cnt = (double)HW;
  const double mean = (t1 + cnt * p1) / (cnt * cpg);
  const double m2 = t2 - 2.0 * mean * t1 + 2.0 * u + cnt * (cpg * mean * mean - 2.0 * mean * p1 + p2);
  const float meanf = (float)mean;
  const float var = (float)(m2 / (cnt * cpg));
  const float rstd = 1.0f / sqrtf(snap_relu(var) + eps);
  for (int cc = lane; cc < cpg; cc += 64) {
    mu[(int64_t)n * C + c_lo + cc] = meanf;
    sc[(int64_t)n * C + c_lo + cc] = rstd * gamma[c_lo + cc];
    if (rstd_out) rstd_out[(int64_t)n * C + c_lo + cc] = rstd;
  }
}

__global__ __launch_bounds__(256) void gn_finalize_tiled_kernel(
    const float* __restrict__ partial, int S, int HW, int C, int groups, float eps,
    const float* __restrict__ gamma, float* __restrict__ mu, float* __restrict__ sc,
    float* __restrict__ rstd_out, int tile_rows) {
  __shared__ double wsum[4][2];
  const int i = blockIdx.x;
  const int n = i / groups, g = i - n * groups;
  const int cpg = C / groups;
  const int c_lo = g * cpg;
  const int live = tile_rows < 0 ? S
                   : (int)((((int64_t)(n + 1) * HW - 1) / tile_rows) - (((int64_t)n * HW) / tile_rows)) + 1;
  const int count = live * cpg;
  const float gam = (int)threadIdx.x < cpg ? gamma[c_lo + threadIdx.x] : 0.f;
  double t1 = 0.0, t2 = 0.0;
  int e = threadIdx.x;
  for (; e + 768 < count; e += 1024) {
    float2 v[4];
#pragma unroll
    for (int u = 0; u < 4; ++u) {
      const int ee = e + 256 * u;
      const int s = ee / cpg, cc = ee - s * cpg;
      v[u] = *reinterpret_cast<const float2*>(partial + (((int64_t)n * S + s) * C + c_lo + cc) * 2);
    }
#pragma unroll
    for (int u = 0; u < 4; ++u) {
      t1 += (double)v[u].x;
      t2 += (double)v[u].y;
    }
  }
  for (; e < count; e += 256) {
    const int s = e / cpg, cc = e - s * cpg;
    const float* pp = partial + (((int64_t)n * S + s) * C + c_lo + cc) * 2;
    t1 += (double)pp[0];
    t2 += (double)pp[1];
  }
  t1 = wave_sum_f64(t1);
  t2 = wave_sum_f64(t2);
  if ((threadIdx.x & 63) == 0) { wsum[threadIdx.x >> 6][0] = t1; wsum[threadIdx.x >> 6][1] = t2; }
  __syncthreads();
  t1 = ((wsum[0][0] + wsum[1][0]) + wsum[2][0]) + wsum[3][0];
  t2 = ((wsum[0][1] + wsum[1][1]) + wsum[2][1]) + wsum[3][1];
  const double cnt = (double)HW;
  const double mean = t1 / (cnt * cpg);
  const double m2 = t2 - 2.0 * mean * t1 + cnt * (cpg * mean * mean);
  const float meanf = (float)mean;
  const float var = (float)(m2 / (cnt * cpg));
  const float rstd = 1.0f / sqrtf(snap_relu(var) + eps);
  for (int cc = threadIdx.x; cc < cpg; cc += 256) {
    mu[(int64_t)n * C + c_lo + cc] = meanf;
    sc[(int64_t)n * C + c_lo + cc] = rstd * (cc < 256 ? gam : gamma[c_lo + cc]);
    if (rstd_out) rstd_out[(int64_t)n * C + c_lo + cc] = rstd;
  }
}

__global__ void gn_apply_kernel(const float* __restrict__ x, float* __restrict__ y, int64_t total4,
                                int HW, int C, const float* __restrict__ mu,
                                const float* __restrict__ sc, const float* __restrict__ beta,
                                int mode) {
  const int64_t i = (int64_t)blockIdx.x * blockDim.x + threadIdx.x;
  if (i >= total4) return;
  const int C4 = C >> 2;
  const int q = (int)(i % C4);
  const int64_t pix = i / C4;
  const int n = (int)(pix / HW);
  const f32x4 v = reinterpret_cast<const f32x4*>(x)[i];
  const f32x4 m = *reinterpret_cast<const f32x4*>(mu + (int64_t)n * C + 4 * q);
  const f32x4 s = *reinterpret_cast<const f32x4*>(sc + (int64_t)n * C + 4 * q);
  const f32x4 b = *reinterpret_cast<const f32x4*>(beta + 4 * q);
  f32x4 o;
#pragma unroll
  for (int e = 0; e < 4; ++e) {
    if (mode == SNAP_PRO_GN_RELU)
      o[e] = snap_relu((v[e] - m[e]) * s[e] + b[e]);
    else
      o[e] = (snap_relu(v[e]) - m[e]) * s[e] + b[e];
  }
  reinterpret_cast<f32x4*>(y)[i] = o;
}

__global__ void max_pool_kernel(const float* __restrict__ x, float* __restrict__ y, int N, int H,
                                int W, int C, int Ho, int Wo) {
  const int C4 = C >> 2;
  const int64_t total = (int64_t)N * Ho * Wo * C4;
  const int64_t i = (int64_t)blockIdx.x * blockDim.x + threadIdx.x;
  if (i >= total) return;
  const int q = (int)(i % C4);
  int64_t r = i / C4;
  const int wo = (int)(r % Wo); r /= Wo;
  const int ho = (int)(r % Ho);
  const int n = (int)(r / Ho);
  f32x4 best = {-INFINITY, -INFINITY, -INFINITY, -INFINITY};
#pragma unroll
  for (int dh = 0; dh < 3; ++dh) {
    const int hi = ho * 2 - 1 + dh;
    if (hi < 0 || hi >= H) continue;
#pragma unroll
    for (int dw = 0; dw < 3; ++dw) {
      const int wi = wo * 2 - 1 + dw;
      if (wi < 0 || wi >= W) continue;
      const f32x4 v =
          *reinterpret_cast<const f32x4*>(x + (((int64_t)n * H + hi) * W + wi) * C + 4 * q);
#pragma unroll
      for (int e = 0; e < 4; ++e) best[e] = snap_max_nan(best[e], v[e]);
    }
  }
  reinterpret_cast<f32x4*>(y)[i] = best;
}

struct GnPlan { int S, ppb; };
inline GnPlan gn_plan(int N, int HW, int C) {
  const int chunks = (C + 1023) / 1024;
  int S = (1024 + N * chunks - 1) / (N * chunks);
  const int smax = (HW + 7) / 8;
  if (S > smax) S = smax;
  if (S > 256) S = 256;
  if (S < 1) S = 1;
  GnPlan p;
  p.ppb = (HW + S - 1) / S;
  p.S = (HW + p.ppb - 1) / p.ppb;
  return p;
}

}

extern "C" int snap_weight_standardize_f32(const float* w, float* out, int32_t K, int32_t Cout,
                                           float eps, void* stream) {
  if (!w || !out) return SNAP_ERR_NULL;
  if (K <= 0 || Cout <= 0) return SNAP_ERR_BAD_SHAPE;
  hipLaunchKernelGGL(weight_std_kernel, dim3((unsigned)snap_cdiv(Cout, WS_COLS)), dim3(1024), 0,
                     static_cast<hipStream_t>(stream), w, out, K, Cout, eps);
// ... 136 lines not shown
```

### snap_amd/models/image_encoder.py

```python
import numpy as np
import torch

from snap_amd import autograd as ag
from snap_amd import ops
from snap_amd.configs import defaults as default_configs
from snap_amd.models import base
from snap_amd.models import resnet
from snap_amd.models import types
from snap_amd.models import vit


def pad_to_multiple(images, stride, channel_pad=0):
  if isinstance(images, (list, tuple)):
    parts = list(images)
    shape = np.array(parts[0].shape[-3:-1])
    pad = stride - shape % stride
    native = all(p.is_cuda and p.is_contiguous() and p.dim() == 4 and not base.needs_grad(p) for p in parts)
    if native and ops.NATIVE_GLUE and all(p.shape[1:] == parts[0].shape[1:] for p in parts):
      H, W, C = parts[0].shape[1:]
      out = torch.empty((sum(p.shape[0] for p in parts), H + int(pad[0]), W + int(pad[1]), C + int(channel_pad)),
                        dtype=torch.float32, device=parts[0].device)
      n0 = 0
      for p in parts:
        ops.pad_image(p, int(pad[0]), int(pad[1]), int(channel_pad), out=out[n0:n0 + p.shape[0]])
# ... 18 lines not shown
  def init_params(self, gen, device):
    params = {}
    for level, c in enumerate(self.in_dims):
      params[f'{level}_skip_norm'] = {
          'scale': torch.ones(1, 1, 1, c, device=device),
          'bias': torch.zeros(1, 1, 1, c, device=device),
      }
      params[f'{level}_skip_conv'] = {
          'kernel': base.lecun_normal(gen, (1, 1, c, self.output_dim), c, device)
      }
    return params

  def __call__(self, params, input_features, train=False):
    assert len(input_features) == self.num_levels
    out_features = []
    f_prev = None
    for level, f_skip in enumerate(input_features):
      norm = params[f'{level}_skip_norm']
      kernel = params[f'{level}_skip_conv']['kernel']
      if f_prev is not None:
        assert f_skip.shape[-3] == f_prev.shape[-3] * 2, "Image heights don't match."
        assert f_skip.shape[-2] == f_prev.shape[-2] * 2, "Image widths don't match."
      if base.needs_grad(f_skip, kernel, norm['scale'], f_prev):
        f = ag.conv2d(f_skip, kernel, prologue=ops.PRO_RELU_GN,
                      gn_params=(norm['scale'], norm['bias']), up_prev=f_prev)
      else:
        mu, sc = ops.group_norm_stats(f_skip, norm['scale'].reshape(-1), relu_first=True)
        f = ops.conv2d(
            f_skip, kernel, prologue=ops.PRO_RELU_GN,
            gn=(mu, sc, norm['bias'].reshape(-1)), up_prev=f_prev,
        )
      f_prev = f
      out_features.append(f)
    return out_features


class ImageEncoder(base.Module):

  def __init__(self, config, dtype=torch.float32, in_channels=3):
    self.config = config
    num_pyr_levels = config.num_pyr_levels
    self.is_vit = config.encoder_name == 'vit'
    if self.is_vit:
      self.encoder = vit.ViTEncoder(config.encoder, config.output_dim, dtype)
      self.decoder = None
      return
    if config.encoder_name != 'resnet':
      raise ValueError(config.encoder_name)
    self.encoder = resnet.ResNetV2(config.encoder, dtype, in_channels=in_channels)
    if num_pyr_levels is None:
      num_pyr_levels = len(self.encoder.level_names)
    self.max_stride = (not config.encoder.skip_root_block) * 2 + num_pyr_levels - 1
    self.level_names = self.encoder.level_names[:num_pyr_levels][::-1]
    width = self.encoder.width
    in_dims = [width * 4 * 2 ** (int(n[5:]) - 1) for n in self.level_names]
    self.decoder = FPNDecoder(config.output_dim, num_pyr_levels, in_dims, dtype)

  def init_params(self, gen, device):
    if self.is_vit:
      return {'encoder': self.encoder.init_params(gen, device)}
    return {
        'encoder': self.encoder.init_params(gen, device),
        'decoder': self.decoder.init_params(gen, device),
    }

  def __call__(self, params, image, train=False, ctx=None, rng=None):
    parts = [im.to(torch.float32) for im in image] if isinstance(image, (list, tuple)) else [image.to(torch.float32)]
    input_shape = np.array(parts[0].shape[-3:-1])
    if self.is_vit or len(parts) == 1:
      image = parts[0] if len(parts) == 1 else torch.cat(parts, 0)
    else:
      image = parts
    if self.is_vit:
      patch = self.config.encoder.patch_size
      padded = vit.pad_to_patch(image, patch)
      f = self.encoder(params['encoder'], padded, train=train, ctx=ctx)
      h, w = np.ceil(input_shape / patch).astype(int)
      return types.FeatureImagePyramid(
          features=[f[..., :h, :w, :]], strides=[np.array([patch, patch], dtype=np.float64)])
    rgb4 = (parts[0].shape[-1] == 3 and ops.precision() in ops.SPLIT_PARTS
            and not any(base.needs_grad(p) for p in parts) and not train)
    image_padded = pad_to_multiple(image, 2**self.max_stride, channel_pad=1 if rgb4 else 0).contiguous()
    padded_shape = np.array(image_padded.shape[-3:-1])
    encoder_features = self.encoder(params['encoder'], image_padded, train=train, ctx=ctx)
    skip_features = []
    for layer_name in self.level_names:
      _, f = sorted(encoder_features[layer_name].items())[-1]
      skip_features.append(f)
    out_features = self.decoder(params['decoder'], skip_features, train=train)
    strides = [padded_shape / np.array(f.shape[-3:-1]) for f in out_features]
    crops = []
    for s, f in zip(strides, out_features):
      h, w = np.round(np.ceil(input_shape / s)).astype(int)
      crops.append(f[..., :h, :w, :])
    return types.FeatureImagePyramid(features=crops, strides=strides)

  default_config = staticmethod(default_configs.image_encoder)
```

### snap_amd/models/resnet.py

```python
import torch

from snap_amd import autograd as ag
from snap_amd import ops
from snap_amd.configs import defaults as default_configs
from snap_amd.models import base


def get_block_desc(depth):
  if isinstance(depth, list):
    depth = tuple(depth)
  return {
      26: [2, 2, 2, 2],
      50: [3, 4, 6, 3],
      101: [3, 4, 23, 3],
      152: [3, 8, 36, 3],
      200: [3, 24, 36, 3],
  }.get(depth, depth)


def _std(ctx, kernel):
  if base.needs_grad(kernel):
    pre = getattr(ctx, 'pre_std', None)
    if pre is not None and id(kernel) in pre:
      return pre[id(kernel)]
    return ag.weight_standardize(kernel)
  return ctx.standardized(kernel, ops.weight_standardize)


def _kernels(tree, out):
  for k, v in tree.items():
    if isinstance(v, dict):
      _kernels(v, out)
    elif k == 'kernel':
      out.append(v)
  return out


def _conv_gn(ctx, x, kernel, gn_p, gn_stats=None, emit=True, presplit=False, **kw):
  w = _std(ctx, kernel)
  mode = None if not emit else ('both' if emit == 'both' else 'raw')
  if base.needs_grad(x, w, gn_p['scale'], gn_p['bias']):
    return ag.conv2d(x, w, prologue=ops.PRO_GN_RELU, gn_params=(gn_p['scale'], gn_p['bias']),
                     emit_gn_stats='raw' if emit else None, **kw)
  if presplit and ops.USE_PRESPLIT and gn_stats is None and w.shape[2] % 16 == 0:
    xs = ops.gn_norm_split(x, gn_p['scale'].reshape(-1), gn_p['bias'].reshape(-1))
    if xs is not None:
      return ops.conv2d(xs, w, emit_gn_stats=mode, **kw)
  return ops.conv2d(x, w, prologue=ops.PRO_GN_RELU, gn=gn_stats or _gn(x, gn_p),
                    emit_gn_stats=mode, **kw)


SHARE_PROJ_GN = True
FORK_SHORTCUT = True


def _gn(x, p, relu_first=False):
  mu, sc = ops.group_norm_stats(x, p['scale'].reshape(-1), relu_first=relu_first)
  return mu, sc, p['bias'].reshape(-1)


def residual_unit(ctx, p, x, stride, nmid, last_of_stage=False):
  nmid = nmid or x.shape[-1] // 4
  nout = nmid * 4
  train = base.needs_grad(x, p['conv1']['kernel'])
  gn1 = None if train else _gn(x, p['gn1'])
  proj = x.shape[-1] != nout or stride != 1
  if train and proj and SHARE_PROJ_GN and x.shape[-1] % 4 == 0 and x.shape[-1] == p['conv1']['kernel'].shape[2]:
    y, residual = ag.conv2d_shared_gn(x, _std(ctx, p['conv1']['kernel']), _std(ctx, p['conv_proj']['kernel']),
                                      (p['gn1']['scale'], p['gn1']['bias']), stride2=stride, emit_gn_stats='raw')
    y = _conv_gn(ctx, y, p['conv2']['kernel'], p['gn2'], stride=stride, padding=((1, 1), (1, 1)), presplit=True)
    return _conv_gn(ctx, y, p['conv3']['kernel'], p['gn3'], residual=residual, presplit=True,
                    emit='both' if (last_of_stage and ops.GN_STATS_BOTH) else True)
  if train and FORK_SHORTCUT:
    y, xs = _conv_gn(ctx, x, p['conv1']['kernel'], p['gn1'], gn1, fork_input=True)
  else:
    y, xs = None, x
  if x.shape[-1] != nout or stride != 1:
    residual = _conv_gn(ctx, xs, p['conv_proj']['kernel'], p['gn1'], gn1, emit=False, stride=stride)
  else:
    residual = xs
  if y is None:
    y = _conv_gn(ctx, x, p['conv1']['kernel'], p['gn1'], gn1)
  y = _conv_gn(ctx, y, p['conv2']['kernel'], p['gn2'], stride=stride, padding=((1, 1), (1, 1)),
               presplit=True)
  y = _conv_gn(ctx, y, p['conv3']['kernel'], p['gn3'], residual=residual, presplit=True,
               emit='both' if (last_of_stage and ops.GN_STATS_BOTH) else True)
  return y


def _init_unit(gen, device, cin, nmid, stride):
  nout = nmid * 4
  def gn(c):
    return {'scale': torch.ones(1, 1, 1, c, device=device),
            'bias': torch.zeros(1, 1, 1, c, device=device)}
  def conv(kh, kw, ci, co):
    return {'kernel': base.lecun_normal(gen, (kh, kw, ci, co), kh * kw * ci, device)}
  p = {'gn1': gn(cin), 'conv1': conv(1, 1, cin, nmid), 'gn2': gn(nmid),
       'conv2': conv(3, 3, nmid, nmid), 'gn3': gn(nmid),
       'conv3': conv(1, 1, nmid, nout)}
  if cin != nout or stride != 1:
    p['conv_proj'] = conv(1, 1, cin, nout)
  return p


class ResNetV2(base.Module):

  def __init__(self, config, dtype=torch.float32, in_channels=3):
    self.config = config
    self.in_channels = in_channels
    self.blocks = get_block_desc(config.depth)
    if config.limit_num_blocks is not None:
      self.blocks = self.blocks[: config.limit_num_blocks]
    self.level_names = [f'stage{i + 1}' for i in range(len(self.blocks))]
    self.width = int(64 * config.width)
    if self.width % 32 != 0:
      raise ValueError('GroupNorm(32) needs the base width to be a multiple of 32')

  def init_params(self, gen, device):
    w = self.width
    params = {}
    if self.config.skip_root_block:
      c = self.in_channels
      params['conv_root'] = {'kernel': base.lecun_normal(gen, (3, 3, c, w), 9 * c, device)}
    else:
      c = self.in_channels
      params['root_block'] = {
          'conv_root': {'kernel': base.lecun_normal(gen, (7, 7, c, w), 49 * c, device)}
      }
    cin = w
    for i, size in enumerate(self.blocks):
      nmid = w * 2**i
      stage = {}
      for u in range(size):
        stride = 2 if (u == 0 and i > 0) else 1
        stage[f'unit{u + 1:02d}'] = _init_unit(gen, device, cin, nmid, stride)
        cin = nmid * 4
      params[f'block{i + 1}'] = stage
    return params

  def __call__(self, params, image, *, train=False, ctx=None, rng=None):
    ctx = ctx or base.ForwardContext()
    out = {}
    kernels = _kernels(params, [])
    if base.needs_grad(*kernels):
      pre = dict(getattr(ctx, 'pre_std', None) or {})
      std = ag.weight_standardize_multi(kernels)
      pre.update({id(k): s for k, s in zip(kernels, std)})
      ctx.pre_std = pre
      if ops.precision() in ops.HALF_MATH:
        ops.pack_weights_bf16_multi(list(std), math=ops.precision())
    else:
      ctx.standardize_all(kernels, ops.weight_standardize_multi)
      if ops.precision() in ops.SPLIT_PARTS:
        ops.pack_weights_split_multi([ctx._lookup(k) for k in kernels], ops.precision())
    w_root = params['conv_root' if self.config.skip_root_block else 'root_block']
    w_root = w_root['kernel'] if self.config.skip_root_block else w_root['conv_root']['kernel']
    cin_kw = {'cin': w_root.shape[2]} if image.shape[-1] != w_root.shape[2] else {}
    if self.config.skip_root_block:
      w = _std(ctx, params['conv_root']['kernel'])
      conv = ag.conv2d if base.needs_grad(w) else ops.conv2d
      x = conv(image, w, padding=((1, 1), (1, 1)), prologue=ops.PRO_AFFINE, in_affine=(2.0, -1.0),
               emit_gn_stats='raw', **cin_kw)
    else:
      w = _std(ctx, params['root_block']['conv_root']['kernel'])
      conv = ag.conv2d if base.needs_grad(w) else ops.conv2d
      x = conv(image, w, stride=2, padding=((3, 3), (3, 3)), prologue=ops.PRO_AFFINE,
               in_affine=(2.0, -1.0), **cin_kw)
      pool = ag.max_pool_3x3s2 if base.needs_grad(x) else ops.max_pool_3x3s2
      x = out['stem'] = pool(x)
    for i, size in enumerate(self.blocks):
      stage = {}
      nmid = self.width * 2**i
      for u in range(size):
        name = f'unit{u + 1:02d}'
        stride = 2 if (u == 0 and i > 0) else 1
        x = stage[name] = residual_unit(ctx, params[f'block{i + 1}'][name], x, stride, nmid,
                                        last_of_stage=u + 1 == size)
      out[f'stage{i + 1}'] = stage
    return out

  default_config = staticmethod(default_configs.resnet)
```

### snap_amd/ops.py

```python
import contextlib
import sys
import ctypes
import threading
import typing
import weakref
import os

import numpy as np
import torch

from snap_amd import _lib

PRO_NONE, PRO_AFFINE, PRO_GN_RELU, PRO_RELU_GN, PRO_RELU = 0, 1, 2, 3, 4
EPI_BIAS, EPI_RELU, EPI_RESIDUAL, EPI_UPSAMPLE2X_ADD, EPI_ROWMASK, EPI_GELU = 1, 2, 4, 8, 16, 32
POOLING = {'max': 0, 'sum': 1, 'mean': 2}
SIM_CHUNK = 64



_TUNING_DEFAULTS = {
    'OVERLAP_AERIAL': True,
    'POOLED_SPLIT': True,
    'CLASS_ROWS': True,
    'LIFT_IN_CONSUMER': True,
    'MLP_GATHER_XCD_GROUP': 8,
    'NATIVE_GLUE': True,
    'USE_PRESPLIT': False,
    'CONV_TILE': None,
    'CONV_BK': None,
    'CONV_NO_HALO': False,
    'CONV_NO_RS': False,
    'CONV_RS_NSPLIT': 0,
    'CONV_RS_FORCE': False,
    'CONV_NO_WS': False,
    'SPLITK_STATS': True,
    'CONV_NO_PLAIN': False,
    'USE_PRESPLIT_VOTING': True,
    'PS_RES_INIT': True,
    'PS_TILE': 0,
    'BF16_PS': True,
    'USE_FUSED_GN_STATS': True,
    'GN_STATS_BOTH': True,
    'USE_SPLITK': True,
    'FUSED_TEMPLATE_PACK': True,
    'SIM_GENERAL_KERNEL': False,
    'LATTICE_WINDOW': True,
    'WGRAD_SIDE_STREAM': True,
}


class Tuning:
  __slots__ = tuple(_TUNING_DEFAULTS)

  def __init__(self, **kw):
    for k, v in _TUNING_DEFAULTS.items():
      object.__setattr__(self, k, kw.pop(k, v))
    if kw:
      raise TypeError(f'Tuning: unknown switch(es) {sorted(kw)}')

  def replace(self, **kw):
    vals = {k: getattr(self, k) for k in _TUNING_DEFAULTS}
    for k in kw:
      if k not in vals:
        raise TypeError(f'Tuning: unknown switch {k!r}')
    vals.update(kw)
    return Tuning(**vals)

  def __repr__(self):
    diff = {k: getattr(self, k) for k, v in _TUNING_DEFAULTS.items() if getattr(self, k) != v}
    return 'Tuning(' + ', '.join(f'{k}={v!r}' for k, v in diff.items()) + ')'


_DEFAULT_TUNING = Tuning()
_TUNING_TLS = threading.local()


def tuning():
  t = getattr(_TUNING_TLS, 'tuning', None)
  return _DEFAULT_TUNING if t is None else t


@contextlib.contextmanager
def tuning_scope(base=None, **overrides):
  prev = getattr(_TUNING_TLS, 'tuning', None)
  _TUNING_TLS.tuning = (base if base is not None else tuning()).replace(**overrides)
  try:
    yield _TUNING_TLS.tuning
  finally:
    _TUNING_TLS.tuning = prev


_raw_stream = getattr(torch._C, '_cuda_getCurrentRawStream', None)
_raw_device = getattr(torch._C, '_cuda_getDevice', None)


def _stream():
  if _raw_stream is not None and _raw_device is not None:
    return ctypes.c_void_p(_raw_stream(_raw_device()))
  return ctypes.c_void_p(torch.cuda.current_stream().cuda_stream)


_SIDE_STREAMS = {}


def side_stream(device=None):
  idx = torch.cuda.current_device() if device is None else torch.device(device).index
  if idx is None:
    idx = torch.cuda.current_device()
  s = _SIDE_STREAMS.get(idx)
  if s is None:
    s = _SIDE_STREAMS[idx] = torch.cuda.Stream(device=idx)
  return s


class KernelProfiler:

  def __init__(self):
    self.records = {}

  def region(self, name, flops=0.0, nbytes=0.0, tag=None):
    return _Region(self, name, flops, nbytes, tag)

  def launches(self, name):
    torch.cuda.synchronize()
    return [
# ... 201 lines not shown
  return PreSplit(out, shape)


def _stationary_mode(T=None):
  T = tuning() if T is None else T
  if T.CONV_NO_RS:
    return 1
  if T.CONV_RS_FORCE:
    return 4 if T.CONV_NO_WS else 2
  return 3 if T.CONV_NO_WS else 0


class PackedWeights:

  def __init__(self, data, shape):
    self.data = data
    self.shape = tuple(int(v) for v in shape)

  def numel(self):
    return int(np.prod(self.shape))


def pack_stacked_templates_split(templates, S):
  lib = _lib.load()
  _f32(templates, 'templates')
  R, H, W, D = templates.shape
  KH, KW, RS = H + S - 1, W + S - 1, R * S * S
  nbytes = lib.snap_conv2d_packed_weights_split_bytes(KH * KW, D, RS, 2)
  if nbytes == 0:
    return None
  out = torch.empty(nbytes // 2, dtype=torch.bfloat16, device=templates.device)
  with _region('pack_stacked_templates', 0.0, 4.0 * templates.numel() + float(nbytes)):
    st = lib.snap_pack_stacked_templates_split_bf16(_p(templates), H, W, D, R, S, _p(out), nbytes, _stream())
  _lib.check(st, 'snap_pack_stacked_templates_split_bf16')
  return PackedWeights(out, (KH, KW, D, RS))


HALF_MATH = ('bf16', 'fp16')
SPLIT_PARTS = {'bf16x3': 2, 'bf16x6': 3}


def kernel_image(w_shape, math):
  KH, KW, Cin, Cout = w_shape
  parts = SPLIT_PARTS.get(math, 0)
  if parts and _lib.load().snap_conv2d_packed_weights_split_bytes(KH * KW, Cin, Cout, parts) == 0:
    math, parts = 'f32', 0
  return math, parts, math != 'f32' and Cin >= 4


def conv2d_presplit_supported(x_shape, w_shape, stride=1, padding=((0, 0), (0, 0))):
  lib = _lib.load()
  N, H, W, Cs = x_shape
  KH, KW, Cin, Cout = w_shape
  (pt, pb), (pl, pr) = padding
  if Cs != Cin or Cin % 16:
    return False
  Ho = (H + pt + pb - KH) // stride + 1
  Wo = (W + pl + pr - KW) // stride + 1
  if Ho <= 0 or Wo <= 0:
    return False
  if kernel_image(w_shape, 'bf16x3')[1] != 2:
    return False
  d = _lib.SnapConvDesc(N, H, W, Cin, Cs, KH, KW, stride, pt, pl, Ho, Wo, Cout, Cout, PRO_NONE, 0, 1.0, 0.0)
  return bool(lib.snap_conv2d_presplit_supported(ctypes.byref(d)))


class ConvPlan(typing.NamedTuple):
  desc: _lib.SnapConvDesc
  out_shape: tuple
  out_dtype: torch.dtype
  engine: str
  family: str
  tag: str
  image: str
  parts: int
  extras: bool
  workspace_bytes: int
  stats_bytes: int
  stats_count: int
  stats_relu: bool
  gn_partial_rows: int
  tile_rows: int
  gnb: bool
  w_split_parts: int
  w_split_root: int
  w_half: int
  x_half: int
  x_presplit: int
  ps_tile: int
  ps_res_init: int
  bk_hint: int
  tune_flags: int


def plan_conv(
    x, w, stride=1, padding=((0, 0), (0, 0)), cin=None, prologue=PRO_NONE,
    gn=None, in_affine=(1.0, 0.0), bias=None, relu=False, residual=None,
    up_prev=None, row_mask=None, rows_in=None, rows_out=None, row_count=None, out=None,
    emit_gn_stats=None, math=None, gelu=False, res_init=None, ps_tile=None, out_half=False, out_stride=None,
    gn_bwd_stats=None, bf16_ring=False,
):
  lib = _lib.load()
  T = tuning()
  ps = isinstance(x, PreSplit)
  pw = isinstance(w, PackedWeights)
  xh = (not ps) and x.dtype in (torch.bfloat16, torch.float16)
  no_rows = rows_in is None and rows_out is None and row_count is None
  if xh:
    want = 'fp16' if x.dtype == torch.float16 else 'bf16'
    math = want if math is None else math
    if (math != want or prologue != PRO_NONE or rows_in is not None or x.shape[-1] % 8 or w.shape[2] % 8
        or emit_gn_stats is not None):
      raise ValueError('conv2d: a half-precision input takes the matching engine, prologue NONE, whole '
                       'channel octets, no input row list / statistics')
  if ps:
    if prologue != PRO_NONE or not no_rows or math not in (None, 'bf16x3'):
      raise ValueError('conv2d: a PreSplit input takes prologue NONE, no row lists, math bf16x3')
    math = 'bf16x3'
  if pw and not ps:
    raise ValueError('conv2d: PackedWeights (a two-part split image) go with a PreSplit input')
  N, H, W, Cs = x.shape
  KH, KW, Cin, Cout = w.shape
  if cin is None:
    cin = Cs
  if cin != Cin:
    raise ValueError(f'conv2d: kernel expects Cin={Cin}, input has {cin}')
  (pt, pb), (pl, pr) = padding
  Ho = (H + pt + pb - KH) // stride + 1
  Wo = (W + pl + pr - KW) // stride + 1
  M = N * Ho * Wo
  out_dtype = torch.float32
  if out_half:
    hm = precision() if math is None else math
    if (hm not in HALF_MATH or out is not None or emit_gn_stats is not None or up_prev is not None
        or prologue not in (PRO_NONE, PRO_RELU) or Cs % 4 or Cin < 4 or Cout % 4):
      raise ValueError('conv2d: out_half needs a training-precision engine launch (prologue NONE / RELU, '
                       'no statistics / up-sampling epilogue, channel quads)')
    out_dtype = torch.float16 if hm == 'fp16' else torch.bfloat16
  elif out is not None:
    if out_stride is not None:
      if (out_stride % 4 or out_stride < Cout or out.numel() != M * out_stride or emit_gn_stats is not None
          or residual is not None or up_prev is not None):
        raise ValueError('conv2d: out_stride needs out [rows, out_stride], out_stride % 4 == 0, a plain epilogue')
    elif out.numel() != M * Cout:
      raise ValueError('conv2d: out has the wrong size')
  if out_stride is not None and out is None:
    raise ValueError('conv2d: out_stride goes with out')
  epi = 0
  if prologue in (PRO_GN_RELU, PRO_RELU_GN):
    mu, sc, beta = gn
    if mu.numel() != N * Cin or sc.numel() != N * Cin or beta.numel() != Cin:
      raise ValueError('conv2d: GroupNorm statistics have the wrong size')
  if bias is not None:
    epi |= EPI_BIAS
    if bias.numel() != Cout:
      raise ValueError('conv2d: bias size')
  if relu:
    epi |= EPI_RELU
  if gelu:
    epi |= EPI_GELU
  if residual is not None:
    epi |= EPI_RESIDUAL
    y_shape = (N, Ho, Wo, Cout) if out is None else tuple(out.shape)
    if tuple(residual.shape) != y_shape:
      raise ValueError(f'conv2d: residual {tuple(residual.shape)} vs {y_shape}')
  if up_prev is not None:
    epi |= EPI_UPSAMPLE2X_ADD
    if tuple(up_prev.shape) != (N, Ho // 2, Wo // 2, Cout):
      raise ValueError('conv2d: up_prev shape')
  if row_mask is not None:
    epi |= EPI_ROWMASK
    if row_mask.numel() != M:
      raise ValueError('conv2d: row_mask size')
  tile_hint = 1000000 * _stationary_mode(T)
  if T.CONV_TILE:
    bm, bn = (int(v) for v in T.CONV_TILE.split('x'))
    tile_hint += bm * 1000 + bn
  d = _lib.SnapConvDesc(
      N, H, W, Cin, Cs, KH, KW, stride, pt, pl, Ho, Wo, Cout, Cout if out_stride is None else int(out_stride), prologue,
      epi, float(in_affine[0]), float(in_affine[1]), tile_hint,
  )
  dref = ctypes.byref(d)
  math = precision() if math is None else math
  if math not in ENGINES:
    raise ValueError(f'conv2d: math={math!r}')
  math, parts, packed = kernel_image((KH, KW, Cin, Cout), math)
  packed = packed and Cs % 4 == 0
  qparts = parts if packed and not ps else 0
  ps1 = bool(bf16_ring and xh and x.dtype == torch.bfloat16 and math == 'bf16' and T.BF16_PS and Cs == Cin and Cin % 16 == 0
             and rows_out is None and row_count is None and up_prev is None and gn_bwd_stats is None
             and out is None and Cout % 4 == 0 and lib.snap_conv2d_presplit_supported(dref))
  if xh and out_half and not ps1:
    raise ValueError('conv2d: a half-precision input AND output need the one-part pre-split engine (bf16, Cin % 16 == 0, '
                     'no row lists)')
  kind = lib.snap_conv2d_stationary_kind(dref, qparts) if (qparts == 2 and no_rows) else 0
  pst = (T.PS_TILE if ps_tile is None else int(ps_tile)) if (ps or ps1) else 0
  wbytes = sbytes = scount = rows32 = tile_rows = 0
  gnb = False
  if no_rows:
    if ps:
      wbytes = lib.snap_conv2d_presplit_workspace_bytes(dref, pst) if T.USE_SPLITK else 0
    elif not (ps1 or kind or out_half):
      wbytes = lib.snap_conv2d_workspace_bytes(dref) if T.USE_SPLITK else 0
    if wbytes:
      half_engine = math in HALF_MATH and packed and Cin % 4 == 0 and not ps
      if emit_gn_stats is not None and (qparts >= 2 or half_engine) and T.SPLITK_STATS:
        sbytes = lib.snap_conv2d_splitk_gn_partial_bytes(dref)
        if sbytes:
          scount, rows32, tile_rows = 1, 32, 32
    elif (gn_bwd_stats is not None and xh and emit_gn_stats is None and out is None and up_prev is None
          and not relu and not gelu and row_mask is None):
      gx, gmu, grs, gga, gbe, gmode = gn_bwd_stats
      pbytes = lib.snap_conv2d_gn_partial_bytes_ex(dref, 0)
      if (pbytes and tuple(gx.shape) == (N, Ho, Wo, Cout) and gmu.numel() == N * Cout and grs.numel() == N * Cout
          and gga.numel() == Cout and gbe.numel() == Cout and gmode in (PRO_GN_RELU, PRO_RELU_GN)):
        sbytes, scount, gnb = pbytes, 1, True
        tile_rows = lib.snap_conv2d_tile_rows_ex(dref, 0)
    elif emit_gn_stats is not None:
      sbytes = (lib.snap_conv2d_presplit_gn_partial_bytes(dref, pst) if ps
                else lib.snap_conv2d_gn_partial_bytes_ex(dref, qparts))
      if sbytes:
        scount = 2 if (emit_gn_stats == 'both' and math in SPLIT_PARTS) else 1
        tile_rows = lib.snap_conv2d_presplit_tile_rows(dref, pst) if ps else lib.snap_conv2d_tile_rows_ex(dref, qparts)
  if ps and (parts != 2 or Cin % 16):
    raise ValueError('conv2d: the pre-split engine needs Cin % 16 == 0 and a two-part weight image')
  family, image, iparts = 'conv_igemm', None, 0
  root = xpre = res0 = 0
  if (parts and (KH, KW, stride, Cin, Cs) == (7, 7, 2, 3, 4) and (pt, pl) == (3, 3)
      and prologue in (PRO_NONE, PRO_AFFINE) and no_rows and not sbytes and not ps):
    family, image, iparts, root = f'conv_split_{math}', math + '/root', parts, 1
  elif ps1:
    family, image, iparts, xpre = 'conv_bf16', 'bf16/ps1', 1, 1
  elif packed:
    family = f'conv_split_{math}' if parts else ('conv_fp16' if math == 'fp16' else 'conv_bf16')
    image, iparts = math, parts
    if ps:
      xpre, res0 = 1, int(T.PS_RES_INIT if res_init is None else bool(res_init))
  bk_hint = tune_flags = 0
  tuned = bool(T.CONV_BK or T.CONV_NO_HALO or T.CONV_RS_NSPLIT or T.CONV_NO_PLAIN)
  if tuned:
    bk_hint = int(T.CONV_BK or 0)
    tune_flags = int(bool(T.CONV_NO_HALO)) | 8 * int(bool(T.CONV_NO_PLAIN)) | ((int(T.CONV_RS_NSPLIT) & 15) << 4)
  return ConvPlan(
      desc=d, out_shape=(N, Ho, Wo, Cout), out_dtype=out_dtype, engine=math if image else 'f32', family=family,
      tag='PS_' if ps else 'PS1_' if ps1 else ('', 'RS_', 'WS_', 'WS_')[kind], image=image, parts=iparts,
      extras=bool(not no_rows or wbytes or sbytes or image or tuned), workspace_bytes=wbytes,
      stats_bytes=sbytes, stats_count=scount, stats_relu=bool(sbytes) and emit_gn_stats == 'relu',
      gn_partial_rows=rows32, tile_rows=tile_rows, gnb=gnb,
      w_split_parts=iparts, w_split_root=root, w_half=int(image == 'fp16'), x_half=int(xh and not ps1),
      x_presplit=xpre, ps_tile=pst if xpre else 0, ps_res_init=res0, bk_hint=bk_hint, tune_flags=tune_flags)


def conv2d(
    x, w, *, stride=1, padding=((0, 0), (0, 0)), cin=None, prologue=PRO_NONE,
    gn=None, in_affine=(1.0, 0.0), bias=None, relu=False, residual=None,
    up_prev=None, row_mask=None, rows_in=None, rows_out=None, row_count=None, out=None,
    emit_gn_stats=None, math=None, gelu=False, res_init=None, ps_tile=None, out_half=False, out_stride=None,
    gn_bwd_stats=None, bf16_ring=False,
):
  lib = _lib.load()
  ps = isinstance(x, PreSplit)
  pw = isinstance(w, PackedWeights)
  if ps:
    xd = _chk(x.data, torch.bfloat16, 'x')
  else:
    xd = _chk(x, x.dtype if x.dtype in (torch.bfloat16, torch.float16) else torch.float32, 'x')
  wd = w.data if pw else _f32(w, 'w')
  if out is not None:
    _f32(out, 'out')
  for t, nm in ((rows_in, 'rows_in'), (rows_out, 'rows_out'), (row_count, 'row_count')):
    if t is not None:
      _chk(t, torch.int32, nm)
  mu = sc = beta = None
  if prologue in (PRO_GN_RELU, PRO_RELU_GN):
    mu, sc, beta = gn
    _f32(mu, 'gn_mu'); _f32(sc, 'gn_sc'); _f32(beta, 'gn_beta')
  if bias is not None:
    _f32(bias, 'bias')
  if residual is not None:
    _f32(residual, 'residual')
  if up_prev is not None:
    _f32(up_prev, 'up_prev')
  if row_mask is not None:
    _mask(row_mask, 'row_mask')
  p = plan_conv(x, w, stride, padding, cin, prologue, gn, in_affine, bias, relu, residual, up_prev, row_mask, rows_in,
                rows_out, row_count, out, emit_gn_stats, math, gelu, res_init, ps_tile, out_half, out_stride,
                gn_bwd_stats, bf16_ring)
  dev = xd.device
  y = out if out is not None else torch.empty(p.out_shape, dtype=p.out_dtype, device=dev)
  kws = torch.empty(p.workspace_bytes // 4, dtype=torch.float32, device=dev) if p.workspace_bytes else None
  partial = torch.empty(p.stats_bytes // 4, dtype=torch.float32, device=dev) if p.stats_count else None
  partial2 = torch.empty(p.stats_bytes // 4, dtype=torch.float32, device=dev) if p.stats_count == 2 else None
  wpk = None
  if p.image is not None:
    wpk = wd if pw else _packed_weights(w, p.image, p.parts)
  ex = None
  if p.extras:
    ex = _lib.SnapConvExtras()
    if rows_in is not None or rows_out is not None or row_count is not None:
      ex.rows_in, ex.rows_out, ex.row_count = _pv(rows_in), _pv(rows_out), _pv(row_count)
    if kws is not None:
      ex.workspace, ex.workspace_bytes = kws.data_ptr(), p.workspace_bytes
    if partial is not None:
      ex.gn_partial, ex.gn_partial_bytes = partial.data_ptr(), p.stats_bytes
      ex.gn_partial_relu, ex.gn_partial_rows = int(p.stats_relu), p.gn_partial_rows
    if partial2 is not None:
      ex.gn_partial2, ex.gn_partial2_bytes = partial2.data_ptr(), p.stats_bytes
    if p.gnb:
      for t, nm in zip(gn_bwd_stats[:5], ('gn_bwd x', 'gn_bwd mu', 'gn_bwd rstd', 'gn_bwd gamma', 'gn_bwd beta')):
        _f32(t, nm)
      ex.gnb_x, ex.gnb_mu, ex.gnb_rstd, ex.gnb_gamma, ex.gnb_beta = (t.data_ptr() for t in gn_bwd_stats[:5])
      ex.gnb_mode = int(gn_bwd_stats[5])
    if wpk is not None:
      ex.w_bf16, ex.w_bf16_bytes = wpk.data_ptr(), wpk.numel() * 2
      ex.w_split_parts, ex.w_split_root, ex.w_half, ex.x_half = p.w_split_parts, p.w_split_root, p.w_half, p.x_half
      ex.x_presplit, ex.ps_tile, ex.ps_res_init = p.x_presplit, p.ps_tile, p.ps_res_init
      if out_half:
        ex.y_half = y.data_ptr()
    ex.bk_hint, ex.tune_flags = p.bk_hint, p.tune_flags
  N, Ho, Wo, Cout = p.out_shape
  KH, KW, Cin = w.shape[:3]
  M = N * Ho * Wo
  kflops = 2.0 * KH * KW * Cin * Cout
  if row_count is None:
    flops = kflops * M
    nbytes = 4.0 * ((x.numel() if ps else x.numel() * (0.5 if p.x_half or p.image == 'bf16/ps1' else 1.0)) + w.numel() + y.numel()
                    + (residual.numel() if residual is not None else 0))
  else:
    flops = lambda: kflops * int(row_count.item())
    nbytes = lambda: 4.0 * (int(row_count.item()) * (Cin + Cout) + wd.numel())
  with _region(
      p.family, flops, nbytes,
      lambda: f'{p.tag}M{M}{"r" if row_count is not None else ""}_K{KH}x{KW}x{Cin}_N{Cout}_s{stride}_p{prologue}_e{p.desc.epilogue}',
  ):
    st = lib.snap_conv2d_nhwc_ex_f32(
        ctypes.byref(p.desc), _p(xd), _p(wd), None if out_half else _p(y), _p(mu), _p(sc), _p(beta), _p(bias),
        _p(residual), _p(up_prev), _p(row_mask), None if ex is None else ctypes.byref(ex),
        _stream(),
    )
  _lib.check(st, 'snap_conv2d_nhwc_ex_f32')
  if p.gnb:
    y._snap_gnb_partial = (partial, p.tile_rows, gn_bwd_stats[0].data_ptr(), gn_bwd_stats[0]._version, int(gn_bwd_stats[5]))
  elif partial is not None:
    y._snap_gn_partial = (partial, p.tile_rows, p.stats_relu)
    if partial2 is not None and ex.gn_partial2_done:
      y._snap_gn_partial_relu = (partial2, p.tile_rows, True)
  return y


def pack_weights_bf16(w, half=False):
  lib = _lib.load()
  _f32(w, 'w')
  KH, KW, Cin, Cout = w.shape
  nbytes = lib.snap_conv2d_packed_weights_bytes(KH * KW, Cin, Cout)
  out = torch.empty(nbytes // 2, dtype=torch.float16 if half else torch.bfloat16, device=w.device)
  fn = lib.snap_conv2d_pack_weights_f16 if half else lib.snap_conv2d_pack_weights_bf16
  st = fn(_p(w), KH * KW, Cin, Cout, _p(out), nbytes, _stream())
  _lib.check(st, 'snap_conv2d_pack_weights_f16' if half else 'snap_conv2d_pack_weights_bf16')
  return out


PACK_EPOCH = 0


def _image_get(w, key, explicit=False):
  slot = getattr(w, '_snap_packed', None)
  hit = None if slot is None else slot.get(key)
  if isinstance(hit, tuple):
    return hit[2] if hit[0] == PACK_EPOCH and hit[1] == w._version else None
  return hit if explicit else None


def _image_put(w, key, image):
  slot = getattr(w, '_snap_packed', None)
  if slot is None:
    slot = w._snap_packed = {}
  slot[key] = (PACK_EPOCH, w._version, image)


def _packed_weights(w, math, parts):
  wpk = _image_get(w, math, explicit=True)
  if wpk is None:
    if math.endswith('/root'):
      wpk = pack_weights_split_root_bf16(w, parts)
    else:
      wpk = pack_weights_split_bf16(w, parts) if parts else pack_weights_bf16(w, half=(math == 'fp16'))
    try:
      _image_put(w, math, wpk)
    except AttributeError:
      pass
  return wpk


def pack_weights_split_bf16(w, parts):
  lib = _lib.load()
  _f32(w, 'w')
  KH, KW, Cin, Cout = w.shape
  nbytes = lib.snap_conv2d_packed_weights_split_bytes(KH * KW, Cin, Cout, parts)
  out = torch.empty(nbytes // 2, dtype=torch.bfloat16, device=w.device)
  st = lib.snap_conv2d_pack_weights_split_bf16(_p(w), KH * KW, Cin, Cout, parts, _p(out), nbytes,
                                               _stream())
  _lib.check(st, 'snap_conv2d_pack_weights_split_bf16')
  return out


def pack_weights_split_root_bf16(w, parts):
  lib = _lib.load()
  _f32(w, 'w')
  if tuple(w.shape[:3]) != (7, 7, 3):
    raise ValueError('pack_weights_split_root_bf16: w must be [7, 7, 3, Cout]')
  Cout = w.shape[3]
  nbytes = lib.snap_conv2d_packed_weights_split_root_bytes(Cout, parts)
  out = torch.empty(nbytes // 2, dtype=torch.bfloat16, device=w.device)
  st = lib.snap_conv2d_pack_weights_split_root_bf16(_p(w), Cout, parts, _p(out), nbytes, _stream())
  _lib.check(st, 'snap_conv2d_pack_weights_split_root_bf16')
  return out


_PACK_ITEM = np.dtype([('w', np.uint64), ('out', np.uint64), ('taps', np.int32), ('Cin', np.int32),
                       ('Cout', np.int32), ('block_begin', np.int32)])


def pack_weights_split_multi(ws, math):
  parts = SPLIT_PARTS[math]
  lib = _lib.load()
  todo = [w for w in ws if _image_get(w, math) is None and kernel_image(w.shape, math)[2]]
  if not todo:
    return
  items = np.zeros(len(todo), dtype=_PACK_ITEM)
  outs = []
# ... 284 lines not shown


_WSTD_ITEM = np.dtype([('w', '<u8'), ('dws', '<u8'), ('out', '<u8'), ('K', '<i4'), ('Cout', '<i4'),
                       ('block_begin', '<i4'), ('reserved', '<i4')])


def _wstd_table(ws, dwss, outs, cols=32):
  items = np.zeros(len(ws), dtype=_WSTD_ITEM)
  blk = 0
  for i, w in enumerate(ws):
    _f32(w, 'w'); _f32(outs[i], 'out')
    K = w.shape[0] * w.shape[1] * w.shape[2]
    items[i] = (w.data_ptr(), 0 if dwss is None else _f32(dwss[i], 'dws').data_ptr(),
                outs[i].data_ptr(), K, w.shape[3], blk, 0)
    blk += (w.shape[3] + cols - 1) // cols
  table = upload_table(items, ws[0].device)
  return table, blk


def weight_standardize_multi(ws, eps=1e-10):
  lib = _lib.load()
  outs = [torch.empty_like(w) for w in ws]
  table, blocks = _wstd_table(ws, None, outs, cols=32)
  with _region('weight_standardize', 0.0, 16.0 * sum(w.numel() for w in ws)):
    st = lib.snap_weight_standardize_multi_f32(_p(table), len(ws), blocks, eps, _stream())
  _lib.check(st, 'snap_weight_standardize_multi_f32')
  return outs


def weight_standardize_bwd_multi(ws, dwss, eps=1e-10):
  lib = _lib.load()
  outs = [torch.empty_like(w) for w in ws]
  table, blocks = _wstd_table(ws, dwss, outs)
  st = lib.snap_weight_standardize_bwd_multi_f32(_p(table), len(ws), blocks, eps, _stream())
  _lib.check(st, 'snap_weight_standardize_bwd_multi_f32')
  return outs


MATMUL_PRECISION = 'f32'
ENGINES = ('f32', 'bf16', 'fp16', 'bf16x3', 'bf16x6')
_ENGINE_TLS = threading.local()


def precision():
  e = getattr(_ENGINE_TLS, 'engine', None)
  return MATMUL_PRECISION if e is None else e


@contextlib.contextmanager
def engine_scope(engine, tuning=None):
  if tuning is not None:
    with tuning_scope(tuning):
      with engine_scope(engine):
        yield
    return
  if engine is None:
    yield
    return
  if engine not in ENGINES:
    raise ValueError(f'engine {engine!r}: expected one of {ENGINES}')
  prev = getattr(_ENGINE_TLS, 'engine', None)
  _ENGINE_TLS.engine = engine
  try:
    yield
  finally:
    _ENGINE_TLS.engine = prev


def engine_of_dtype(dtype):
  if dtype in (torch.float16, 'float16', 'fp16'):
    return 'fp16'
  if dtype in (torch.bfloat16, 'bfloat16', 'bf16'):
    return 'bf16'
  if dtype in (torch.float32, 'float32', 'f32', None):
    return None
  raise ValueError(f'dtype {dtype!r}: expected float32 | float16 | bfloat16')


def group_norm_stats(x, gamma, *, groups=32, eps=1e-5, relu_first=False, want_rstd=False):
  lib = _lib.load()
  _f32(x, 'x'); _f32(gamma, 'gamma')
  N, H, W, C = x.shape
  HW = H * W
  wsb = lib.snap_group_norm_stats_workspace_bytes(N, HW, C, groups)
  ws = torch.empty(wsb // 4 + 4, dtype=torch.float32, device=x.device)
  mu = torch.empty((N, C), dtype=torch.float32, device=x.device)
  sc = torch.empty((N, C), dtype=torch.float32, device=x.device)
  rstd = torch.empty((N, C), dtype=torch.float32, device=x.device) if want_rstd else None
  fused = getattr(x, '_snap_gn_partial', None)
  if fused is not None and fused[2] != bool(relu_first):
    fused = getattr(x, '_snap_gn_partial_relu', None) if relu_first else None
  if fused is not None and fused[2] == bool(relu_first) and groups == 32 and tuning().USE_FUSED_GN_STATS:
    partial, tile_rows, _ = fused
    with _region('group_norm_stats', 0.0, 4.0 * partial.numel()):
      st = lib.snap_group_norm_stats_from_partial_f32(
          _p(partial), N, HW, C, groups, eps, tile_rows, _p(gamma), _p(mu), _p(sc), _p(rstd),
          _stream(),
      )
    _lib.check(st, 'snap_group_norm_stats_from_partial_f32')
    return (mu, sc, rstd) if want_rstd else (mu, sc)
  with _region('group_norm_stats', 0.0, 8.0 * x.numel()):
    st = lib.snap_group_norm_stats_f32(
        _p(x), N, HW, C, C, groups, eps, int(relu_first), _p(gamma), _p(mu),
        _p(sc), _p(rstd), _p(ws), ws.numel() * 4, _stream(),
    )
  _lib.check(st, 'snap_group_norm_stats_f32')
  if want_rstd:
    return mu, sc, rstd
  return mu, sc


def group_norm_apply(x, mu, sc, beta, mode):
  lib = _lib.load()
  _f32(x, 'x'); _f32(mu, 'mu'); _f32(sc, 'sc'); _f32(beta, 'beta')
  N, H, W, C = x.shape
  y = torch.empty_like(x)
  st = lib.snap_group_norm_apply_f32(
      _p(x), _p(y), N, H * W, C, _p(mu), _p(sc), _p(beta), mode, _stream()
  )
  _lib.check(st, 'snap_group_norm_apply_f32')
  return y


def pad_image(x, pad_h, pad_w, pad_c=0, out=None):
  lib = _lib.load()
  _f32(x, 'x')
  *lead, H, W, C = x.shape
  N = int(np.prod(lead)) if lead else 1
  shape = (*lead, H + pad_h, W + pad_w, C + pad_c)
  if out is None:
    y = torch.empty(shape, dtype=torch.float32, device=x.device)
  else:
    y = _f32(out, 'out')
    if tuple(y.shape) != tuple(shape):
      raise ValueError(f'pad_image: out {tuple(y.shape)} != {tuple(shape)}')
  st = lib.snap_pad_image_f32(_p(x), N, H, W, C, int(pad_h), int(pad_w), int(pad_c), _p(y), _stream())
  _lib.check(st, 'snap_pad_image_f32')
  return y


def voxel_points(xy, z):
  lib = _lib.load()
  _f32(xy, 'xy'); _f32(z, 'z')
  B, Z = z.shape
  X, Y = xy.shape[-3:-1]
  batched = xy.dim() == 4
  if xy.shape[-1] != 2 or (batched and xy.shape[0] != B):
    raise ValueError('voxel_points: shapes')
  out = torch.empty((B, X, Y, Z, 3), dtype=torch.float32, device=z.device)
  st = lib.snap_voxel_points_f32(_p(xy), int(batched), _p(z), B, X * Y, Z, _p(out), _stream())
  _lib.check(st, 'snap_voxel_points_f32')
  return out


def max_pool_3x3s2(x):
  lib = _lib.load()
  _f32(x, 'x')
  N, H, W, C = x.shape
  Ho, Wo = (H + 2 - 3) // 2 + 1, (W + 2 - 3) // 2 + 1
  y = torch.empty((N, Ho, Wo, C), dtype=torch.float32, device=x.device)
  st = lib.snap_max_pool_3x3s2_f32(_p(x), _p(y), N, H, W, C, _stream())
  _lib.check(st, 'snap_max_pool_3x3s2_f32')
  return y


def pooled_channels(feature_dim, weighted=True, use_variance=True, add_minmax=False):
# ... 629 lines not shown
```

Before: 400.2 scenes/s.

## Finalize GroupNorm statistics inside the producing conv via last-block atomic counters

The conv kernels that already write per-tile GroupNorm partial sums now also bump a per-(sample, column-unit) atomic counter. Whichever block arrives last reduces the partials and writes mean and scale for the next layer's GroupNorm. This removes the separate group_norm_stats finalize launch and its reread of the partials, with the ResNet encoder passing the consumer's gamma down so the producer knows what to compute. In exchange it adds atomics, write-through partial stores and acquire fences, a pooled counter buffer that must return to zero after each use, and a serial tail of work in the last block.

```diff
diff --git a/include/snap_hip.h b/include/snap_hip.h
--- a/include/snap_hip.h
+++ b/include/snap_hip.h
@@ -74,6 +74,16 @@
   const float* gnb_gamma;
   const float* gnb_beta;
   int32_t gnb_mode;
+  float* gn_mu_out;
+  float* gn_sc_out;
+  const float* gn_gamma;
+  float* gn_mu_out2;
+  float* gn_sc_out2;
+  const float* gn_gamma2;
+  int32_t* gn_counters;
+  size_t gn_counter_bytes;
+  float gn_eps;
+  int32_t gn_final_done;
 } SnapConvExtras;
 #define SNAP_TUNE_NO_HALO 1
 #define SNAP_TUNE_NO_PLAIN 8
diff --git a/snap_amd/_lib.py b/snap_amd/_lib.py
--- a/snap_amd/_lib.py
+++ b/snap_amd/_lib.py
@@ -34,6 +34,9 @@
       ('x_presplit', c_int), ('ps_tile', c_int), ('ps_res_init', c_int),
       ('bk_hint', c_int), ('tune_flags', c_int), ('gn_partial_rows', c_int), ('w_half', c_int), ('x_half', c_int), ('y_half', ptr),
       ('gnb_x', ptr), ('gnb_mu', ptr), ('gnb_rstd', ptr), ('gnb_gamma', ptr), ('gnb_beta', ptr), ('gnb_mode', c_int),
+      ('gn_mu_out', ptr), ('gn_sc_out', ptr), ('gn_gamma', ptr), ('gn_mu_out2', ptr), ('gn_sc_out2', ptr),
+      ('gn_gamma2', ptr), ('gn_counters', ptr), ('gn_counter_bytes', c_size), ('gn_eps', c_float),
+      ('gn_final_done', c_int),
   ]
 
 
diff --git a/snap_amd/csrc/conv_common.h b/snap_amd/csrc/conv_common.h
--- a/snap_amd/csrc/conv_common.h
+++ b/snap_amd/csrc/conv_common.h
@@ -5,8 +5,20 @@
 #include <stdlib.h>
 
 #include "common.h"
+#include "gn_finalize.h"
 
 namespace snapconv {
+struct GnFin {
+  float* mu;
+  float* sc;
+  const float* gamma;
+  float* mu2;
+  float* sc2;
+  const float* gamma2;
+  float eps;
+  int32_t* cnt;
+};
+
 struct ConvArgs {
   SnapConvDesc d;
   const float* x;
@@ -33,6 +45,8 @@
   int gn_relu;
   int gn_rows32;
   int gn_slabs;
+  GnFin gn_fin;
+  int32_t* gn_fin_done;
   int M;
   int K;
   int ctiles;
@@ -96,7 +110,71 @@
   return x / (1.0f + __expf(-2.0f * u));
 }
 
-template <int BM, int BN, bool DUAL = false, int NT = 256, bool SKIP_RES = false, int OUTH = 0, bool GNB = false>
+typedef __attribute__((address_space(1))) unsigned long long gu64_t;
+typedef __attribute__((address_space(1))) int gi32_t;
+
+__device__ __forceinline__ void gn_store_partial(float* o, float t1, float t2, bool write_through) {
+  if (write_through) {
+    const unsigned long long bits = ((unsigned long long)__float_as_uint(t2) << 32) | __float_as_uint(t1);
+    __hip_atomic_store((gu64_t*)(o), bits, __ATOMIC_RELAXED, __HIP_MEMORY_SCOPE_AGENT);
+  } else {
+    o[0] = t1;
+    o[1] = t2;
+  }
+}
+
+template <int NT>
+__device__ __forceinline__ void gn_arrive_finalize(const snapconv::GnFin& f, float* partial, float* partial2,
+                                                   int* lds, int N, int HW, int Cout, int n_first, int w0,
+                                                   int w1, int w2, int c0, int unit_cols, int tile_rows,
+                                                   int S) {
+  const int cpg = Cout >> 5;
+  const int u = c0 / unit_cols;
+  const int ucols = min(unit_cols, Cout - u * unit_cols);
+  asm volatile("s_waitcnt vmcnt(0)" ::: "memory");
+  __syncthreads();
+  if (threadIdx.x == 0) {
+    const int w[3] = {w0, w1, w2};
+    int last = 0;
+#pragma unroll
+    for (int k = 0; k < 3; ++k) {
+      const int n = n_first + k;
+      if (w[k] <= 0 || n >= N) continue;
+      const int expected = gn_live_tiles(n, HW, S, tile_rows) * ucols;
+      const int old = __hip_atomic_fetch_add((gi32_t*)(f.cnt + n * 32 + u), w[k], __ATOMIC_RELAXED,
+                                             __HIP_MEMORY_SCOPE_AGENT);
+      if (old + w[k] == expected) last |= 1 << k;
+    }
+    if (last) {
+      __builtin_amdgcn_fence(__ATOMIC_ACQUIRE, "agent");
+      asm volatile("s_waitcnt vmcnt(0)" ::: "memory");
+    }
+    lds[0] = last;
+  }
+  __syncthreads();
+  const int last = lds[0];
+  if (last == 0) return;
+  const int lane = threadIdx.x & 63, wv = threadIdx.x >> 6;
+  const int g_lo = (u * unit_cols) / cpg, ng = ucols / cpg;
+  for (int k = 0; k < 3; ++k) {
+    if (!((last >> k) & 1)) continue;
+    const int n = n_first + k;
+    for (int j = wv; j < 2 * ng; j += NT / 64) {
+      const int kind = j >= ng ? 1 : 0;
+      const int g = g_lo + j - kind * ng;
+      const float* gamma = kind ? f.gamma2 : f.gamma;
+      const float* src = kind ? partial2 : partial;
+      if (gamma == nullptr || src == nullptr) continue;
+      gn_finalize_group_wave(src, S, HW, Cout, f.eps, gamma, kind ? f.mu2 : f.mu, kind ? f.sc2 : f.sc, tile_rows,
+                             n, g, lane);
+    }
+    if (threadIdx.x == 0)
+      __hip_atomic_store((gi32_t*)(f.cnt + n * 32 + u), 0, __ATOMIC_RELAXED, __HIP_MEMORY_SCOPE_AGENT);
+  }
+}
+
+template <int BM, int BN, bool DUAL = false, int NT = 256, bool SKIP_RES = false, int OUTH = 0, bool GNB = false,
+          bool FIN = false>
 __device__ __forceinline__ void conv_epilogue(const ConvArgs& a,
                                               f32x16 (&acc)[BM / (NT / 4)][BN / 64],
                                               float* smem, int m0, int n0, int Meff, int row_t,
@@ -256,6 +334,7 @@
   if (want_stats) {
     constexpr int RG = NT / Q;
     const int q = tid % Q, rg = tid / Q;
+    const bool fin = FIN && a.gn_fin.cnt != nullptr;
     for (int pass = 0; pass < (want_relu_too ? 2 : 1); ++pass) {
     float* const dst_partial = pass ? a.gn_partial2 : a.gn_partial;
     __syncthreads();
@@ -281,9 +360,23 @@
       }
       const int slab = row_t - (int)(((int64_t)n * HoWo) / BM);
       float* o = dst_partial + (((int64_t)n * a.gn_slabs + slab) * d.Cout + col) * 2;
-      o[0] = t1;
-      o[1] = t2;
-    }
+      if constexpr (FIN) {
+        gn_store_partial(o, t1, t2, fin);
+      } else {
+        o[0] = t1;
+        o[1] = t2;
+      }
+    }
+    }
+    if constexpr (FIN) {
+      if (fin) {
+        const int unit_cols = (BN % (d.Cout >> 5) == 0 && d.Cout % BN == 0) ? BN : d.Cout;
+        const int wcols = min(BN, d.Cout - n0);
+        const bool second = m0 + BM > m_split && m_split < Meff;
+        gn_arrive_finalize<NT>(a.gn_fin, a.gn_partial, want_relu_too ? a.gn_partial2 : nullptr,
+                               reinterpret_cast<int*>(smem), d.N, HoWo, d.Cout, n_first, m0 < Meff ? wcols : 0,
+                               second ? wcols : 0, 0, n0, unit_cols, BM, a.gn_slabs);
+      }
     }
   }
 }
@@ -341,7 +434,7 @@
     const float* __restrict__ partial, int S, int64_t M, int Cout, int epi,
     const float* __restrict__ bias, const float* __restrict__ residual,
     const uint8_t* __restrict__ row_mask, float* __restrict__ y, int HoWo, int N, int gn_slabs,
-    int gn_relu, float* __restrict__ gn_partial) {
+    int gn_relu, float* gn_partial, const snapconv::GnFin fin) {
   __shared__ float red[256 * 16];
   const int Q = Cout >> 2;
   const int QW = Q < 256 ? Q : 256;
@@ -441,11 +534,15 @@
             t1 += red[(pp * QW + tq) * 16 + sl * 8 + e];
             t2 += red[(pp * QW + tq) * 16 + sl * 8 + 4 + e];
           }
-          o[2 * e] = t1;
-          o[2 * e + 1] = t2;
-        }
-      }
-    }
+          gn_store_partial(o + 2 * e, t1, t2, fin.cnt != nullptr);
+        }
+      }
+    }
+  }
+  if (fin.cnt != nullptr) {
+    const bool second = m0 + 32 > m_split && m_split < M;
+    gn_arrive_finalize<256>(fin, gn_partial, nullptr, reinterpret_cast<int*>(red), N, HoWo, Cout, n_first, Cout,
+                            second ? Cout : 0, 0, 0, Cout, 32, gn_slabs);
   }
 }
 
@@ -456,7 +553,7 @@
     hipLaunchKernelGGL(splitk_reduce_stats_kernel, dim3((unsigned)snap_cdiv((int64_t)a.M, 32)), dim3(256), 0, s,
                        (const float*)a.kpartial, a.ksplit, (int64_t)a.M, a.d.Cout, a.d.epilogue, a.bias,
                        a.residual, a.row_mask, a.y, a.d.Ho * a.d.Wo, a.d.N, (a.d.Ho * a.d.Wo) / 32 + 2,
-                       a.gn_relu, a.gn_partial);
+                       a.gn_relu, a.gn_partial, a.gn_fin);
   } else {
     const int64_t total4 = (int64_t)a.M * (a.d.Cout / 4);
     hipLaunchKernelGGL(splitk_reduce_kernel, dim3((unsigned)snap_cdiv(total4, 256)), dim3(256), 0, s,
diff --git a/snap_amd/csrc/conv_igemm.hip b/snap_amd/csrc/conv_igemm.hip
--- a/snap_amd/csrc/conv_igemm.hip
+++ b/snap_amd/csrc/conv_igemm.hip
@@ -352,7 +352,7 @@
 
   }
 
-  conv_epilogue<BM, BN>(a, acc, smem, m0, n0, Meff, row_t, split);
+  conv_epilogue<BM, BN, false, 256, false, 0, false, true>(a, acc, smem, m0, n0, Meff, row_t, split);
 }
 
 
@@ -628,6 +628,22 @@
     a.gn_partial2_done = const_cast<int32_t*>(&ex->gn_partial2_done);
     *a.gn_partial2_done = 0;
   }
+  a.gn_fin = snapconv::GnFin{nullptr, nullptr, nullptr, nullptr, nullptr, nullptr, 0.f, nullptr};
+  a.gn_fin_done = nullptr;
+  snapconv::GnFin fin = a.gn_fin;
+  if (ex) const_cast<SnapConvExtras*>(ex)->gn_final_done = 0;
+  if (ex && ex->gn_counters) {
+    const bool k1 = ex->gn_gamma != nullptr, k2 = ex->gn_gamma2 != nullptr;
+    if (!gn_partial || ex->gnb_mode || (!k1 && !k2) || (k1 && (!ex->gn_mu_out || !ex->gn_sc_out)) ||
+        (k2 && (!ex->gn_mu_out2 || !ex->gn_sc_out2 || !ex->gn_partial2)))
+      return SNAP_ERR_NULL;
+    if (desc->Cout % 32 != 0 || !(ex->gn_eps >= 0.f)) return SNAP_ERR_BAD_SHAPE;
+    if ((reinterpret_cast<uintptr_t>(ex->gn_counters) & 15) ||
+        ex->gn_counter_bytes < (size_t)desc->N * 32 * sizeof(int32_t))
+      return SNAP_ERR_WORKSPACE;
+    fin = snapconv::GnFin{ex->gn_mu_out, ex->gn_sc_out, ex->gn_gamma, ex->gn_mu_out2, ex->gn_sc_out2,
+                          ex->gn_gamma2, ex->gn_eps, ex->gn_counters};
+  }
   a.kpartial = ex ? static_cast<float*>(ex->workspace) : nullptr;
   a.kpartial_bytes = ex ? ex->workspace_bytes : 0;
   if (reinterpret_cast<uintptr_t>(a.kpartial) & 15) a.kpartial = nullptr;
@@ -723,7 +739,16 @@
     if (ex->w_bf16_bytes < need) return SNAP_ERR_WORKSPACE;
     if (parts) a.cin8 = (d.Cin + 15) / 16 * 16;
     if (reinterpret_cast<uintptr_t>(a.w_bf16) & 15) return SNAP_ERR_BAD_SHAPE;
+    if (parts && fin.cnt) {
+      a.gn_fin = fin;
+      a.gn_fin_done = &const_cast<SnapConvExtras*>(ex)->gn_final_done;
+      *a.gn_fin_done = 1;
+    }
     return parts ? snapconv::launch_split(a, parts, s) : snapconv::launch_bf16(a, s);
   }
+  if (fin.cnt) {
+    a.gn_fin = fin;
+    const_cast<SnapConvExtras*>(ex)->gn_final_done = 1;
+  }
   return vec ? launch_tile<true>(a, s) : launch_tile<false>(a, s);
 }
diff --git a/snap_amd/csrc/conv_split.hip b/snap_amd/csrc/conv_split.hip
--- a/snap_amd/csrc/conv_split.hip
+++ b/snap_amd/csrc/conv_split.hip
@@ -320,7 +320,7 @@
     __syncthreads();
   }
 
-  conv_epilogue<BM, BN, DUAL>(a, acc, smem, m0, n0, Meff, row_t, split);
+  conv_epilogue<BM, BN, DUAL, 256, false, 0, false, true>(a, acc, smem, m0, n0, Meff, row_t, split);
 }
 
 template <int BN, int PRO, int NS, int HPMAX>
@@ -553,7 +553,7 @@
       bcur ^= 1;
     }
   }
-  conv_epilogue<BM, BN>(a, acc, smem, m0, n0, Meff, row_t, split);
+  conv_epilogue<BM, BN, false, 256, false, 0, false, true>(a, acc, smem, m0, n0, Meff, row_t, split);
 }
 
 template <int BN, int PRO, int NS, int HPMAX>
@@ -825,6 +825,10 @@
 int snapconv::launch_split(ConvArgs a, int parts, hipStream_t s) {
   const int kind = stationary_kind(a.d, parts, a.rows_in || a.rows_out || a.row_count);
   if (kind && a.gn_partial && a.gn_rows32) return SNAP_ERR_WORKSPACE;
+  if (kind) {
+    a.gn_fin.cnt = nullptr;
+    if (a.gn_fin_done) *a.gn_fin_done = 0;
+  }
   switch (kind) {
     case 1: return launch_rs(a, s);
     case 2: case 3: return launch_bs(a, s);
diff --git a/snap_amd/csrc/encoder_ops.hip b/snap_amd/csrc/encoder_ops.hip
--- a/snap_amd/csrc/encoder_ops.hip
+++ b/snap_amd/csrc/encoder_ops.hip
@@ -1,4 +1,5 @@
 #include "common.h"
+#include "gn_finalize.h"
 
 namespace {
 
@@ -188,12 +189,6 @@
     o[0] = a1;
     o[1] = a2;
   }
-}
-
-__device__ __forceinline__ double wave_sum_f64(double v) {
-#pragma unroll
-  for (int o = 32; o > 0; o >>= 1) v += __shfl_xor(v, o, 64);
-  return v;
 }
 
 __global__ __launch_bounds__(256) void gn_finalize_kernel(
@@ -254,20 +249,14 @@
   const int n = i / groups, g = i - n * groups;
   const int cpg = C / groups;
   const int c_lo = g * cpg;
-  const int live = tile_rows < 0 ? S
-                   : (int)((((int64_t)(n + 1) * HW - 1) / tile_rows) - (((int64_t)n * HW) / tile_rows)) + 1;
-  const int count = live * cpg;
+  const int count = gn_live_tiles(n, HW, S, tile_rows) * cpg;
   const float gam = (int)threadIdx.x < cpg ? gamma[c_lo + threadIdx.x] : 0.f;
   double t1 = 0.0, t2 = 0.0;
   int e = threadIdx.x;
   for (; e + 768 < count; e += 1024) {
     float2 v[4];
 #pragma unroll
-    for (int u = 0; u < 4; ++u) {
-      const int ee = e + 256 * u;
-      const int s = ee / cpg, cc = ee - s * cpg;
-      v[u] = *reinterpret_cast<const float2*>(partial + (((int64_t)n * S + s) * C + c_lo + cc) * 2);
-    }
+    for (int u = 0; u < 4; ++u) v[u] = gn_partial_entry(partial, S, C, cpg, c_lo, n, e + 256 * u);
 #pragma unroll
     for (int u = 0; u < 4; ++u) {
       t1 += (double)v[u].x;
@@ -275,23 +264,18 @@
     }
   }
   for (; e < count; e += 256) {
-    const int s = e / cpg, cc = e - s * cpg;
-    const float* pp = partial + (((int64_t)n * S + s) * C + c_lo + cc) * 2;
-    t1 += (double)pp[0];
-    t2 += (double)pp[1];
+    const float2 v = gn_partial_entry(partial, S, C, cpg, c_lo, n, e);
+    t1 += (double)v.x;
+    t2 += (double)v.y;
   }
   t1 = wave_sum_f64(t1);
   t2 = wave_sum_f64(t2);
   if ((threadIdx.x & 63) == 0) { wsum[threadIdx.x >> 6][0] = t1; wsum[threadIdx.x >> 6][1] = t2; }
   __syncthreads();
-  t1 = ((wsum[0][0] + wsum[1][0]) + wsum[2][0]) + wsum[3][0];
-  t2 = ((wsum[0][1] + wsum[1][1]) + wsum[2][1]) + wsum[3][1];
-  const double cnt = (double)HW;
-  const double mean = t1 / (cnt * cpg);
-  const double m2 = t2 - 2.0 * mean * t1 + cnt * (cpg * mean * mean);
-  const float meanf = (float)mean;
-  const float var = (float)(m2 / (cnt * cpg));
-  const float rstd = 1.0f / sqrtf(snap_relu(var) + eps);
+  const double w1[4] = {wsum[0][0], wsum[1][0], wsum[2][0], wsum[3][0]};
+  const double w2[4] = {wsum[0][1], wsum[1][1], wsum[2][1], wsum[3][1]};
+  float meanf, rstd;
+  gn_tiled_finish(w1, w2, HW, cpg, eps, meanf, rstd);
   for (int cc = threadIdx.x; cc < cpg; cc += 256) {
     mu[(int64_t)n * C + c_lo + cc] = meanf;
     sc[(int64_t)n * C + c_lo + cc] = rstd * (cc < 256 ? gam : gamma[c_lo + cc]);
diff --git a/snap_amd/csrc/gn_finalize.h b/snap_amd/csrc/gn_finalize.h
--- /dev/null
+++ b/snap_amd/csrc/gn_finalize.h
@@ -0,0 +1,82 @@
+#ifndef SNAP_CSRC_GN_FINALIZE_H_
+#define SNAP_CSRC_GN_FINALIZE_H_
+
+#include "common.h"
+
+namespace {
+
+__device__ __forceinline__ double wave_sum_f64(double v) {
+#pragma unroll
+  for (int o = 32; o > 0; o >>= 1) v += __shfl_xor(v, o, 64);
+  return v;
+}
+
+__device__ __forceinline__ int gn_live_tiles(int n, int HW, int S, int tile_rows) {
+  return tile_rows < 0 ? S
+                       : (int)((((int64_t)(n + 1) * HW - 1) / tile_rows) - (((int64_t)n * HW) / tile_rows)) + 1;
+}
+
+__device__ __forceinline__ float2 gn_partial_entry(const float* partial, int S, int C, int cpg, int c_lo,
+                                                   int n, int e) {
+  const int s = e / cpg, cc = e - s * cpg;
+  return *reinterpret_cast<const float2*>(partial + (((int64_t)n * S + s) * C + c_lo + cc) * 2);
+}
+
+__device__ __forceinline__ void gn_tiled_finish(const double (&w1)[4], const double (&w2)[4], int HW, int cpg,
+                                                float eps, float& meanf, float& rstd) {
+  const double t1 = ((w1[0] + w1[1]) + w1[2]) + w1[3];
+  const double t2 = ((w2[0] + w2[1]) + w2[2]) + w2[3];
+  const double cnt = (double)HW;
+  const double mean = t1 / (cnt * cpg);
+  const double m2 = t2 - 2.0 * mean * t1 + cnt * (cpg * mean * mean);
+  meanf = (float)mean;
+  const float var = (float)(m2 / (cnt * cpg));
+  rstd = 1.0f / sqrtf(snap_relu(var) + eps);
+}
+
+__device__ __forceinline__ void gn_finalize_group_wave(const float* partial, int S, int HW, int C, float eps,
+                                                       const float* gamma, float* mu, float* sc, int tile_rows,
+                                                       int n, int g, int lane) {
+  const int cpg = C >> 5;
+  const int c_lo = g * cpg;
+  const int count = gn_live_tiles(n, HW, S, tile_rows) * cpg;
+  double w1[4] = {0.0, 0.0, 0.0, 0.0}, w2[4] = {0.0, 0.0, 0.0, 0.0};
+  int e = lane;
+  for (; e + 448 < count; e += 512) {
+    float2 v[8];
+#pragma unroll
+    for (int u = 0; u < 8; ++u) v[u] = gn_partial_entry(partial, S, C, cpg, c_lo, n, e + 64 * u);
+#pragma unroll
+    for (int u = 0; u < 8; ++u) {
+      w1[u & 3] += (double)v[u].x;
+      w2[u & 3] += (double)v[u].y;
+    }
+  }
+  {
+    float2 v[8];
+#pragma unroll
+    for (int u = 0; u < 8; ++u)
+      v[u] = e + 64 * u < count ? gn_partial_entry(partial, S, C, cpg, c_lo, n, e + 64 * u) : float2{0.f, 0.f};
+#pragma unroll
+    for (int u = 0; u < 8; ++u)
+      if (e + 64 * u < count) {
+        w1[u & 3] += (double)v[u].x;
+        w2[u & 3] += (double)v[u].y;
+      }
+  }
+#pragma unroll
+  for (int k = 0; k < 4; ++k) {
+    w1[k] = wave_sum_f64(w1[k]);
+    w2[k] = wave_sum_f64(w2[k]);
+  }
+  float meanf, rstd;
+  gn_tiled_finish(w1, w2, HW, cpg, eps, meanf, rstd);
+  for (int cc = lane; cc < cpg; cc += 64) {
+    mu[(int64_t)n * C + c_lo + cc] = meanf;
+    sc[(int64_t)n * C + c_lo + cc] = rstd * gamma[c_lo + cc];
+  }
+}
+
+}
+
+#endif
diff --git a/snap_amd/models/image_encoder.py b/snap_amd/models/image_encoder.py
--- a/snap_amd/models/image_encoder.py
+++ b/snap_amd/models/image_encoder.py
@@ -124,7 +124,8 @@
             and not any(base.needs_grad(p) for p in parts) and not train)
     image_padded = pad_to_multiple(image, 2**self.max_stride, channel_pad=1 if rgb4 else 0).contiguous()
     padded_shape = np.array(image_padded.shape[-3:-1])
-    encoder_features = self.encoder(params['encoder'], image_padded, train=train, ctx=ctx)
+    skip_scales = {name: params['decoder'][f'{level}_skip_norm']['scale'] for level, name in enumerate(self.level_names)}
+    encoder_features = self.encoder(params['encoder'], image_padded, train=train, ctx=ctx, skip_scales=skip_scales)
     skip_features = []
     for layer_name in self.level_names:
       _, f = sorted(encoder_features[layer_name].items())[-1]
diff --git a/snap_amd/models/resnet.py b/snap_amd/models/resnet.py
--- a/snap_amd/models/resnet.py
+++ b/snap_amd/models/resnet.py
@@ -36,7 +36,7 @@
   return out
 
 
-def _conv_gn(ctx, x, kernel, gn_p, gn_stats=None, emit=True, presplit=False, **kw):
+def _conv_gn(ctx, x, kernel, gn_p, gn_stats=None, emit=True, presplit=False, emit_for=None, **kw):
   w = _std(ctx, kernel)
   mode = None if not emit else ('both' if emit == 'both' else 'raw')
   if base.needs_grad(x, w, gn_p['scale'], gn_p['bias']):
@@ -45,9 +45,11 @@
   if presplit and ops.USE_PRESPLIT and gn_stats is None and w.shape[2] % 16 == 0:
     xs = ops.gn_norm_split(x, gn_p['scale'].reshape(-1), gn_p['bias'].reshape(-1))
     if xs is not None:
-      return ops.conv2d(xs, w, emit_gn_stats=mode, **kw)
-  return ops.conv2d(x, w, prologue=ops.PRO_GN_RELU, gn=gn_stats or _gn(x, gn_p),
-                    emit_gn_stats=mode, **kw)
+      with ops.gn_readers(*(emit_for or ())):
+        return ops.conv2d(xs, w, emit_gn_stats=mode, **kw)
+  gn = gn_stats or _gn(x, gn_p)
+  with ops.gn_readers(*(emit_for or ())):
+    return ops.conv2d(x, w, prologue=ops.PRO_GN_RELU, gn=gn, emit_gn_stats=mode, **kw)
 
 
 SHARE_PROJ_GN = True
@@ -59,7 +61,11 @@
   return mu, sc, p['bias'].reshape(-1)
 
 
-def residual_unit(ctx, p, x, stride, nmid, last_of_stage=False):
+def residual_unit(ctx, p, x, stride, nmid, last_of_stage=False, next_scales=(None, None)):
+  def scale(t):
+    return None if t is None else t.reshape(-1)
+  both = last_of_stage and ops.GN_STATS_BOTH
+  out_for = (scale(next_scales[0]), scale(next_scales[1])) if both else (scale(next_scales[0]),)
   nmid = nmid or x.shape[-1] // 4
   nout = nmid * 4
   train = base.needs_grad(x, p['conv1']['kernel'])
@@ -80,11 +86,11 @@
   else:
     residual = xs
   if y is None:
-    y = _conv_gn(ctx, x, p['conv1']['kernel'], p['gn1'], gn1)
+    y = _conv_gn(ctx, x, p['conv1']['kernel'], p['gn1'], gn1, emit_for=(scale(p['gn2']['scale']),))
   y = _conv_gn(ctx, y, p['conv2']['kernel'], p['gn2'], stride=stride, padding=((1, 1), (1, 1)),
-               presplit=True)
+               presplit=True, emit_for=(scale(p['gn3']['scale']),))
   y = _conv_gn(ctx, y, p['conv3']['kernel'], p['gn3'], residual=residual, presplit=True,
-               emit='both' if (last_of_stage and ops.GN_STATS_BOTH) else True)
+               emit='both' if both else True, emit_for=out_for)
   return y
 
 
@@ -138,7 +144,7 @@
       params[f'block{i + 1}'] = stage
     return params
 
-  def __call__(self, params, image, *, train=False, ctx=None, rng=None):
+  def __call__(self, params, image, *, train=False, ctx=None, rng=None, skip_scales=None):
     ctx = ctx or base.ForwardContext()
     out = {}
     kernels = _kernels(params, [])
@@ -174,8 +180,11 @@
       for u in range(size):
         name = f'unit{u + 1:02d}'
         stride = 2 if (u == 0 and i > 0) else 1
-        x = stage[name] = residual_unit(ctx, params[f'block{i + 1}'][name], x, stride, nmid,
-                                        last_of_stage=u + 1 == size)
+        nxt = (params[f'block{i + 1}'].get(f'unit{u + 2:02d}') if u + 1 < size
+               else params.get(f'block{i + 2}', {}).get('unit01') if i + 1 < len(self.blocks) else None)
+        x = stage[name] = residual_unit(
+            ctx, params[f'block{i + 1}'][name], x, stride, nmid, last_of_stage=u + 1 == size,
+            next_scales=(None if nxt is None else nxt['gn1']['scale'], (skip_scales or {}).get(f'stage{i + 1}')))
       out[f'stage{i + 1}'] = stage
     return out
 
diff --git a/snap_amd/ops.py b/snap_amd/ops.py
--- a/snap_amd/ops.py
+++ b/snap_amd/ops.py
@@ -41,6 +41,7 @@
     'BF16_PS': True,
     'USE_FUSED_GN_STATS': True,
     'GN_STATS_BOTH': True,
+    'GN_FINALIZE_IN_PRODUCER': True,
     'USE_SPLITK': True,
     'FUSED_TEMPLATE_PACK': True,
     'SIM_GENERAL_KERNEL': False,
@@ -408,6 +409,7 @@
   gn_partial_rows: int
   tile_rows: int
   gnb: bool
+  gn_final: bool
   w_split_parts: int
   w_split_root: int
   w_half: int
@@ -424,7 +426,7 @@
     gn=None, in_affine=(1.0, 0.0), bias=None, relu=False, residual=None,
     up_prev=None, row_mask=None, rows_in=None, rows_out=None, row_count=None, out=None,
     emit_gn_stats=None, math=None, gelu=False, res_init=None, ps_tile=None, out_half=False, out_stride=None,
-    gn_bwd_stats=None, bf16_ring=False,
+    gn_bwd_stats=None, bf16_ring=False, emit_gn_for=None,
 ):
   lib = _lib.load()
   T = tuning()
@@ -573,6 +575,8 @@
       extras=bool(not no_rows or wbytes or sbytes or image or tuned), workspace_bytes=wbytes,
       stats_bytes=sbytes, stats_count=scount, stats_relu=bool(sbytes) and emit_gn_stats == 'relu',
       gn_partial_rows=rows32, tile_rows=tile_rows, gnb=gnb,
+      gn_final=bool(emit_gn_for is not None and any(g is not None for g in emit_gn_for) and sbytes and not gnb
+                    and Cout % 32 == 0 and T.GN_FINALIZE_IN_PRODUCER and T.USE_FUSED_GN_STATS),
       w_split_parts=iparts, w_split_root=root, w_half=int(image == 'fp16'), x_half=int(xh and not ps1),
       x_presplit=xpre, ps_tile=pst if xpre else 0, ps_res_init=res0, bk_hint=bk_hint, tune_flags=tune_flags)
 
@@ -582,11 +586,13 @@
     gn=None, in_affine=(1.0, 0.0), bias=None, relu=False, residual=None,
     up_prev=None, row_mask=None, rows_in=None, rows_out=None, row_count=None, out=None,
     emit_gn_stats=None, math=None, gelu=False, res_init=None, ps_tile=None, out_half=False, out_stride=None,
-    gn_bwd_stats=None, bf16_ring=False,
+    gn_bwd_stats=None, bf16_ring=False, emit_gn_for=None, gn_eps=1e-5,
 ):
   lib = _lib.load()
   ps = isinstance(x, PreSplit)
   pw = isinstance(w, PackedWeights)
+  if emit_gn_for is None and emit_gn_stats is not None:
+    emit_gn_for = getattr(_GN_READERS_TLS, 'scales', None)
   if ps:
     xd = _chk(x.data, torch.bfloat16, 'x')
   else:
@@ -611,7 +617,7 @@
     _mask(row_mask, 'row_mask')
   p = plan_conv(x, w, stride, padding, cin, prologue, gn, in_affine, bias, relu, residual, up_prev, row_mask, rows_in,
                 rows_out, row_count, out, emit_gn_stats, math, gelu, res_init, ps_tile, out_half, out_stride,
-                gn_bwd_stats, bf16_ring)
+                gn_bwd_stats, bf16_ring, emit_gn_for)
   dev = xd.device
   y = out if out is not None else torch.empty(p.out_shape, dtype=p.out_dtype, device=dev)
   kws = torch.empty(p.workspace_bytes // 4, dtype=torch.float32, device=dev) if p.workspace_bytes else None
@@ -645,6 +651,27 @@
         ex.y_half = y.data_ptr()
     ex.bk_hint, ex.tune_flags = p.bk_hint, p.tune_flags
   N, Ho, Wo, Cout = p.out_shape
+  fin = None
+  if p.gn_final:
+    kinds = [(bool(p.stats_relu), emit_gn_for[0])]
+    if len(emit_gn_for) > 1 and partial2 is not None:
+      kinds.append((True, emit_gn_for[1]))
+    fin = []
+    for slot, (relu_kind, g) in enumerate(kinds):
+      if g is None:
+        continue
+      g = _f32(g.reshape(-1), 'emit_gn_for')
+      if g.numel() != Cout:
+        raise ValueError('conv2d: emit_gn_for scale size')
+      t_mu = torch.empty((N, Cout), dtype=torch.float32, device=dev)
+      t_sc = torch.empty((N, Cout), dtype=torch.float32, device=dev)
+      fin.append((slot, relu_kind, g, t_mu, t_sc))
+      if slot == 0:
+        ex.gn_mu_out, ex.gn_sc_out, ex.gn_gamma = t_mu.data_ptr(), t_sc.data_ptr(), g.data_ptr()
+      else:
+        ex.gn_mu_out2, ex.gn_sc_out2, ex.gn_gamma2 = t_mu.data_ptr(), t_sc.data_ptr(), g.data_ptr()
+    counters = _gn_counters(dev, N * 32)
+    ex.gn_counters, ex.gn_counter_bytes, ex.gn_eps = counters.data_ptr(), N * 32 * 4, float(gn_eps)
   KH, KW, Cin = w.shape[:3]
   M = N * Ho * Wo
   kflops = 2.0 * KH * KW * Cin * Cout
@@ -664,7 +691,15 @@
         _p(residual), _p(up_prev), _p(row_mask), None if ex is None else ctypes.byref(ex),
         _stream(),
     )
+  if st != 0 and fin is not None:
+    _drop_gn_counters(dev)
   _lib.check(st, 'snap_conv2d_nhwc_ex_f32')
+  if fin is not None and ex.gn_final_done:
+    done = {}
+    for slot, relu_kind, g, t_mu, t_sc in fin:
+      if slot == 0 or ex.gn_partial2_done:
+        done[relu_kind] = (g, g._version, float(gn_eps), t_mu, t_sc)
+    y._snap_gn_final = done
   if p.gnb:
     y._snap_gnb_partial = (partial, p.tile_rows, gn_bwd_stats[0].data_ptr(), gn_bwd_stats[0]._version, int(gn_bwd_stats[5]))
   elif partial is not None:
@@ -672,6 +707,41 @@
     if partial2 is not None and ex.gn_partial2_done:
       y._snap_gn_partial_relu = (partial2, p.tile_rows, True)
   return y
+
+
+_GN_READERS_TLS = threading.local()
+
+
+@contextlib.contextmanager
+def gn_readers(*scales):
+  prev = getattr(_GN_READERS_TLS, 'scales', None)
+  _GN_READERS_TLS.scales = scales if any(s is not None for s in scales) else None
+  try:
+    yield
+  finally:
+    _GN_READERS_TLS.scales = prev
+
+
+_GN_COUNTER_POOLS = {}
+_GN_COUNTER_WORDS = 1 << 16
+
+
+def _gn_counters(dev, words):
+  words = (int(words) + 3) // 4 * 4
+  key = (dev.index, _stream().value)
+  pool = _GN_COUNTER_POOLS.get(key)
+  if pool is None or pool[0].numel() < words:
+    pool = _GN_COUNTER_POOLS[key] = [torch.zeros(max(_GN_COUNTER_WORDS, words), dtype=torch.int32, device=dev), 0]
+  if pool[1] + words > pool[0].numel():
+    pool[1] = 0
+  out = pool[0][pool[1]:pool[1] + words]
+  pool[1] += words
+  return out
+
+
+def _drop_gn_counters(dev):
+  for key in [k for k in _GN_COUNTER_POOLS if k[0] == dev.index]:
+    del _GN_COUNTER_POOLS[key]
 
 
 def pack_weights_bf16(w, half=False):
@@ -1122,6 +1192,12 @@
   _f32(x, 'x'); _f32(gamma, 'gamma')
   N, H, W, C = x.shape
   HW = H * W
+  fin = getattr(x, '_snap_gn_final', None)
+  if fin is not None and groups == 32 and not want_rstd and tuning().GN_FINALIZE_IN_PRODUCER:
+    hit = fin.get(bool(relu_first))
+    if (hit is not None and hit[0].data_ptr() == gamma.data_ptr() and hit[0].numel() == gamma.numel()
+        and hit[1] == gamma._version and hit[2] == float(eps)):
+      return hit[3], hit[4]
   wsb = lib.snap_group_norm_stats_workspace_bytes(N, HW, C, groups)
   ws = torch.empty(wsb // 4 + 4, dtype=torch.float32, device=x.device)
   mu = torch.empty((N, C), dtype=torch.float32, device=x.device)
```

Result: slower. 393.2 scenes/s (-1.8%).
